# dwofk/fast-depth

Hardware: NVIDIA H100
Metric: depth-maps/sec @224x224 b64 (higher is better)
Workload: dtype f16

## Files before the change

fastdepth_b200/csrc/fd_chain_tc.cu:

```cuda
#include <cuda.h>

#include <cstdio>
#include <cstdlib>
#include <cstring>
#include <new>
#include <string>
#include <vector>

#include "fd_tc_common.cuh"

namespace fd {

constexpr int CH_WORKERS = 16;
constexpr int CH_WARP_TMA = 16;
constexpr int CH_THREADS = 17 * 32;
constexpr int CH_MAX_PASS = 4;
constexpr int CH_MAX_LAYERS = 8, CH_MAX_KB = 8;
constexpr int CH_PITCH = 15, CH_ROWS = 9;
constexpr int CH_BLK = 136 * 128;
constexpr int CH_IN_BYTES = CH_ROWS * CH_PITCH * 128;
constexpr int CH_SB = 4, CH_B_STAGE = 128 * 128;
constexpr int CH_SD = 4, CH_DWP = 9 * 128 + 512;
constexpr int CH_AFF_BYTES = 512 * 8;
constexpr int CH_OFF_ACT = 1024;
constexpr int CH_OFF_B = CH_OFF_ACT + CH_MAX_KB * CH_BLK;
constexpr int CH_OFF_DWP = CH_OFF_B + CH_SB * CH_B_STAGE;
constexpr int CH_OFF_AFF = CH_OFF_DWP + CH_SD * CH_DWP;
constexpr int CH_OFF_BAR = CH_OFF_AFF + 2 * CH_AFF_BYTES;

struct ChainBarriers {
    uint64_t in_full[CH_MAX_KB];
    uint64_t a_full[CH_MAX_KB];
    uint64_t b_full[CH_SB];
    uint64_t b_empty[CH_SB];
    uint64_t dwp_full[CH_SD], dwp_empty[CH_SD];
    uint64_t aff_full[2], aff_empty[2];
    uint64_t mma_done;
    uint64_t halo_full;
    uint64_t act_free;
};
constexpr int CH_SMEM_BYTES = CH_OFF_BAR + (int)sizeof(ChainBarriers) + 1024;

struct ChainLayer {
    int c_in, c_out;
    int kblocks;
    int np;
    int n_pad;
    int aff_bytes;
    const void* dwp;
    const float2* affine;
};

struct ChainParams {
    int n_img, h, w, rows0;
    int n_layers;
    int out_pitch;
    int sleep_ns;
    int n_zero[2];
    void* out;
    ChainLayer L[CH_MAX_LAYERS];
    unsigned long long* trace;
    unsigned char zero_slots[2][48];
};

struct ChainMaps {
    CUtensorMap in;
    CUtensorMap w[CH_MAX_LAYERS];
    CUtensorMap out[2];
};

__device__ __forceinline__ void st_cluster_u32(uint32_t cluster_addr, uint32_t v) {
    asm volatile("st.shared::cluster.b32 [%0], %1;" ::"r"(cluster_addr), "r"(v) : "memory");
}

#define CH_TRACE(row, idx)                                                                                \
    do {                                                                                                  \
        if (p.trace != nullptr && blockIdx.x == 0 && (idx) < 256) p.trace[(row) * 256 + (idx)] = clock64(); \
    } while (0)

template <typename T, bool RELU6>
__global__ void __cluster_dims__(2, 1, 1) __launch_bounds__(CH_THREADS, 1)
chain_tc_kernel(const __grid_constant__ ChainMaps maps, const __grid_constant__ ChainParams p) {
    using MF = MixFma<T>;
    extern __shared__ uint8_t smem_raw[];
    const uint32_t smem_base = (smem_u32(smem_raw) + 1023u) & ~1023u;
    uint8_t* smem = smem_raw + (smem_base - smem_u32(smem_raw));
    ChainBarriers* bars = reinterpret_cast<ChainBarriers*>(smem + CH_OFF_BAR);
    const int warp = threadIdx.x >> 5, lane = threadIdx.x & 31;
    const uint32_t rank = cluster_ctarank();
    const int cluster_id = blockIdx.x >> 1, n_clusters = gridDim.x >> 1;
    const int rows_local = rank == 0 ? p.rows0 : p.h - p.rows0;
    const int row_first = rank == 0 ? 0 : p.rows0;

    if (threadIdx.x == 0) {
        for (int i = 0; i < CH_MAX_KB; ++i) { mbar_init(smem_u32(&bars->in_full[i]), 1); mbar_init(smem_u32(&bars->a_full[i]), CH_WORKERS / 2); }
        for (int i = 0; i < CH_SB; ++i) { mbar_init(smem_u32(&bars->b_full[i]), 1); mbar_init(smem_u32(&bars->b_empty[i]), CH_WORKERS / 4); }
        for (int i = 0; i < CH_SD; ++i) { mbar_init(smem_u32(&bars->dwp_full[i]), 1); mbar_init(smem_u32(&bars->dwp_empty[i]), CH_WORKERS / 2); }
        for (int i = 0; i < 2; ++i) { mbar_init(smem_u32(&bars->aff_full[i]), 1); mbar_init(smem_u32(&bars->aff_empty[i]), CH_WORKERS); }
        mbar_init(smem_u32(&bars->mma_done), 1);
        mbar_init(smem_u32(&bars->halo_full), 1);
        mbar_init(smem_u32(&bars->act_free), 1);
        fence_barrier_init();
    }
    for (int i = threadIdx.x; i < (CH_OFF_B) / 16; i += CH_THREADS) reinterpret_cast<uint4*>(smem)[i] = make_uint4(0u, 0u, 0u, 0u);
    fence_proxy_async();
    if (warp == CH_WARP_TMA && lane == 0) {
        tma_prefetch_desc(&maps.in);
        tma_prefetch_desc(&maps.out[rank]);
        for (int l = 0; l < p.n_layers; ++l) tma_prefetch_desc(&maps.w[l]);
    }
    pdl_launch_dependents();
    pdl_wait_prior_grid();
    cluster_sync_all();

    if (warp == CH_WARP_TMA) {
        if (lane == 0) {
            uint32_t seq = 0;
            for (int img = cluster_id; img < p.n_img; img += n_clusters)
                for (int l = 0; l < p.n_layers; ++l) {
                    const ChainLayer& L = p.L[l];
                    for (int ps = 0; ps < L.np; ++ps)
                        for (int kb = 0; kb < L.kblocks; ++kb, ++seq) {
                            const uint32_t s = seq & (CH_SB - 1), ph = (seq / CH_SB) & 1u;
                            mbar_wait_sleep(smem_u32(&bars->b_empty[s]), ph ^ 1u, (uint32_t)p.sleep_ns);
                            if (kb == 0 && ps == 0 && img == cluster_id) CH_TRACE(10, l);
                            mbar_expect_tx(smem_u32(&bars->b_full[s]), (uint32_t)CH_B_STAGE);
                            tma_load_2d(smem_base + CH_OFF_B + s * CH_B_STAGE, &maps.w[l], smem_u32(&bars->b_full[s]), kb * 64, ps * 128);
                        }
                }
        } else if (lane == 1) {
            uint32_t dseq = 0, lseq = 0;
            for (int img = cluster_id; img < p.n_img; img += n_clusters)
                for (int l = 0; l < p.n_layers; ++l, ++lseq) {
                    const ChainLayer& L = p.L[l];
                    {
                        const uint32_t s = lseq & 1u, ph = (lseq >> 1) & 1u;
                        mbar_wait_sleep(smem_u32(&bars->aff_empty[s]), ph ^ 1u, (uint32_t)p.sleep_ns);
                        mbar_expect_tx(smem_u32(&bars->aff_full[s]), (uint32_t)L.aff_bytes);
                        bulk_load(smem_base + CH_OFF_AFF + s * CH_AFF_BYTES, L.affine, (uint32_t)L.aff_bytes, smem_u32(&bars->aff_full[s]));
                    }
                    for (int kb = 0; kb < L.kblocks; ++kb, ++dseq) {
                        const uint32_t s = dseq & (CH_SD - 1), ph = (dseq / CH_SD) & 1u;
                        mbar_wait_sleep(smem_u32(&bars->dwp_empty[s]), ph ^ 1u, (uint32_t)p.sleep_ns);
                        mbar_expect_tx(smem_u32(&bars->dwp_full[s]), (uint32_t)CH_DWP);
                        bulk_load(smem_base + CH_OFF_DWP + s * CH_DWP, reinterpret_cast<const uint8_t*>(L.dwp) + (size_t)kb * CH_DWP,
                                  (uint32_t)CH_DWP, smem_u32(&bars->dwp_full[s]));
                    }
                }
        } else if (lane == 2) {
            uint32_t it = 0;
            for (int img = cluster_id; img < p.n_img; img += n_clusters, ++it) {
                if (it > 0) mbar_wait_sleep(smem_u32(&bars->act_free), (it - 1u) & 1u, (uint32_t)p.sleep_ns);
                for (int kb = 0; kb < p.L[0].kblocks; ++kb) {
                    mbar_expect_tx(smem_u32(&bars->in_full[kb]), (uint32_t)CH_IN_BYTES);
                    tma_load_4d(smem_base + CH_OFF_ACT + kb * CH_BLK, &maps.in, smem_u32(&bars->in_full[kb]), kb * 64, 0, row_first - 1, img);
                }
            }
        }
    } else {
        const int grp = warp >> 3, wi = warp & 7;
        const bool dw_active = wi < 7;
        const int tx0 = 2 * (dw_active ? wi : 0);
        const int s0 = tx0 - 1;
        uint32_t rd_off[8];
#pragma unroll
        for (int j = 0; j < 8; ++j) rd_off[j] = ((((uint32_t)lane >> 2) ^ ((uint32_t)(s0 + j) & 7u)) << 4) + (((uint32_t)lane & 3u) << 2);
        uint32_t wr_off[2];
#pragma unroll
        for (int ox = 0; ox < 2; ++ox) wr_off[ox] = ((((uint32_t)lane >> 2) ^ ((uint32_t)(tx0 + ox) & 7u)) << 4) + (((uint32_t)lane & 3u) << 2);
        const int nzc = p.n_zero[rank] * 8;
        const uint32_t z_off = (int)threadIdx.x < nzc ? (uint32_t)p.zero_slots[rank][threadIdx.x >> 3] * 128u + ((uint32_t)threadIdx.x & 7u) * 16u : 0u;
        const int rh = (warp >> 2) & 1, ch = warp >> 3, cp = (lane & 3) * 2;
        const bool wg_leader = (warp & 3) == 0 && lane == 0;
        int e_slot[2], e_halo_slot[2], e_last_slot[2];
        bool e_valid[2], e_halo[2];
#pragma unroll
        for (int h = 0; h < 2; ++h) {
            const int m = rh * 64 + (warp & 3) * 16 + (lane >> 2) + 8 * h, e_ty = m >> 4, e_tx = m & 15;
            e_valid[h] = e_ty < rows_local && e_tx < p.w;
            e_slot[h] = (e_ty + 1) * CH_PITCH + e_tx;
            e_last_slot[h] = e_ty * CH_PITCH + e_tx;
            e_halo[h] = e_valid[h] && (rank == 0 ? e_ty == rows_local - 1 : e_ty == 0);
            e_halo_slot[h] = (rank == 0 ? 0 : (p.rows0 + 1) * CH_PITCH) + e_tx;
        }
        const uint32_t peer_act = mapa_u32(smem_base + CH_OFF_ACT, rank ^ 1u);
        const uint32_t peer_halo_full = mapa_u32(smem_u32(&bars->halo_full), rank ^ 1u);
        const uint32_t peer_mma_done = mapa_u32(smem_u32(&bars->mma_done), rank ^ 1u);
        uint32_t dseq_base = 0, lseq = 0, halo_seq = 0, it = 0, bseq = 0, a_par = 0;
        for (int img = cluster_id; img < p.n_img; img += n_clusters, ++it) {
            for (int l = 0; l < p.n_layers; ++l, ++lseq) {
                const ChainLayer& L = p.L[l];
                const bool last = l == p.n_layers - 1;
                const bool tr0 = it == 0 && warp == 0 && lane == 0, tr8 = it == 0 && warp == 8 && lane == 0;
                if (tr0) CH_TRACE(0, l);
                for (int kb = grp; kb < L.kblocks; kb += 2) {
                    uint8_t* blk = smem + CH_OFF_ACT + kb * CH_BLK;
                    if (l == 0) mbar_wait_sleep(smem_u32(&bars->in_full[kb]), it & 1u, (uint32_t)p.sleep_ns);
                    const uint32_t dseq = dseq_base + (uint32_t)kb, ds = dseq & (CH_SD - 1), dph = (dseq / CH_SD) & 1u;
                    mbar_wait(smem_u32(&bars->dwp_full[ds]), dph);
                    const uint8_t* prm = smem + CH_OFF_DWP + ds * CH_DWP;
                    const f32x2 sc = *reinterpret_cast<const f32x2*>(prm + 9 * 128 + lane * 8);
                    const f32x2 bi = *reinterpret_cast<const f32x2*>(prm + 9 * 128 + 256 + lane * 8);
                    const uint8_t* in0 = blk + s0 * 128;
                    uint32_t o[7][2];
                    if (dw_active) {
                        f32x2 acc[7][2];
#pragma unroll
                        for (int a = 0; a < 7; ++a) acc[a][0] = acc[a][1] = 0ull;
                        f32x2 wq[3][3];
#pragma unroll
                        for (int iy = 0; iy < 9; ++iy) {
                            if (iy < 3) {
#pragma unroll
                                for (int kx = 0; kx < 3; ++kx) wq[iy][kx] = MF::widen(*reinterpret_cast<const uint32_t*>(prm + (iy * 3 + kx) * 128 + lane * 4));
                            }
                            f32x2 row[4];
#pragma unroll
                            for (int ix = 0; ix < 4; ++ix) {
                                const int k = iy * CH_PITCH + ix;
                                row[ix] = MF::widen(*reinterpret_cast<const uint32_t*>(in0 + k * 128 + rd_off[k & 7]));
                            }
#pragma unroll
                            for (int oy = 0; oy < 7; ++oy) {
                                const int ky = iy - oy;
                                if (ky < 0 || ky >= 3) continue;
#pragma unroll
                                for (int ox = 0; ox < 2; ++ox)
#pragma unroll
                                    for (int kx = 0; kx < 3; ++kx) ffma2(acc[oy][ox], row[ox + kx], wq[ky][kx]);
                            }
                        }
#pragma unroll
                        for (int oy = 0; oy < 7; ++oy)
#pragma unroll
                            for (int ox = 0; ox < 2; ++ox) o[oy][ox] = MF::template pack_act<RELU6>(ffma2_abc(acc[oy][ox], sc, bi));
                    }
                    __syncwarp();
                    if (tr0 && kb == 0) CH_TRACE(1, l);
                    if (lane == 0) mbar_arrive(smem_u32(&bars->dwp_empty[ds]));
                    asm volatile("bar.sync %0, %1;" ::"r"(1 + grp), "r"(256) : "memory");
                    if (dw_active) {
#pragma unroll
                        for (int oy = 0; oy < 7; ++oy)
#pragma unroll
                            for (int ox = 0; ox < 2; ++ox)
                                *reinterpret_cast<uint32_t*>(blk + (oy * 16 + tx0 + ox) * 128 + wr_off[ox]) = o[oy][ox];
                    }
                    fence_proxy_async();
                    __syncwarp();
                    if (lane == 0) mbar_arrive(smem_u32(&bars->a_full[kb]));
                }
                dseq_base += (uint32_t)L.kblocks;
                if (tr0) CH_TRACE(2, l);
                if (tr8) CH_TRACE(9, l);

                const uint32_t as = lseq & 1u;
                mbar_wait(smem_u32(&bars->aff_full[as]), (lseq >> 1) & 1u);
                const float2* aff = reinterpret_cast<const float2*>(smem + CH_OFF_AFF + as * CH_AFF_BYTES);
                uint32_t pk[CH_MAX_PASS][16];
#pragma unroll
                for (int ps = 0; ps < CH_MAX_PASS; ++ps) {
                    if (ps >= L.np) break;
                    const int col0 = ps * 128 + ch * 64;
                    const bool act = col0 < L.n_pad;
                    float acc[32];
#pragma unroll
                    for (int i = 0; i < 32; ++i) acc[i] = 0.f;
                    for (int kb = 0; kb < L.kblocks; ++kb, ++bseq) {
                        const uint32_t s = bseq & (CH_SB - 1), ph = (bseq / CH_SB) & 1u;
                        mbar_wait(smem_u32(&bars->a_full[kb]), (a_par >> kb) & 1u);
                        mbar_wait(smem_u32(&bars->b_full[s]), ph);
                        if (tr0 && kb == 0 && ps == 0) CH_TRACE(7, l);
                        if (act) {
                            const uint32_t a_lo = sw128_desc_lo(smem_base + CH_OFF_ACT + (uint32_t)kb * CH_BLK + (uint32_t)rh * 8192u);
                            const uint32_t b_lo = sw128_desc_lo(smem_base + CH_OFF_B + s * CH_B_STAGE + (uint32_t)ch * 8192u);
                            wgmma_fence();
#pragma unroll
                            for (int k4 = 0; k4 < 4; ++k4)
                                wgmma_n64<T>(acc, sw128_desc(a_lo + 2u * k4), sw128_desc(b_lo + 2u * k4), (kb > 0 || k4 > 0) ? 1u : 0u);
                            wgmma_commit();
                            wgmma_wait0();
                        }
                        if (wg_leader) mbar_arrive(smem_u32(&bars->b_empty[s]));
                    }
#pragma unroll
                    for (int i = 0; i < 8; ++i) {
                        const int c = col0 + i * 8 + cp;
                        const bool ok = act && col0 + i * 8 < L.n_pad;
                        const float4 af = ok ? *reinterpret_cast<const float4*>(aff + c) : make_float4(0.f, 0.f, 0.f, 0.f);
#pragma unroll
                        for (int h = 0; h < 2; ++h)
                            pk[ps][8 * h + i] = MF::template pack_act<RELU6>(ffma2_abc(f32x2_make(acc[4 * i + 2 * h], acc[4 * i + 2 * h + 1]),
                                                                                        f32x2_make(af.x, af.y), f32x2_make(af.z, af.w)));
                    }
                }
                for (int kb = 0; kb < L.kblocks; ++kb) a_par ^= 1u << kb;
                if (tr0) CH_TRACE(8, l);
                asm volatile("bar.sync %0, %1;" ::"r"(3), "r"(CH_WORKERS * 32) : "memory");
                if (!last) {
                    if (threadIdx.x == 0) mbar_arrive_cluster(peer_mma_done);
                    mbar_wait_cluster(smem_u32(&bars->mma_done), halo_seq & 1u, 0u);
                }
                if (tr0) CH_TRACE(3, l);
#pragma unroll
                for (int ps = 0; ps < CH_MAX_PASS; ++ps) {
                    if (ps >= L.np) break;
                    const int col0 = ps * 128 + ch * 64;
                    if (col0 >= L.n_pad) continue;
                    const uint32_t boff = (uint32_t)(col0 >> 6) * CH_BLK;
#pragma unroll
                    for (int h = 0; h < 2; ++h) {
                        const int w_slot = last ? e_last_slot[h] : e_slot[h];
#pragma unroll
                        for (int i = 0; i < 8; ++i) {
                            if (col0 + i * 8 >= L.n_pad) break;
                            if (e_valid[h])
                                *reinterpret_cast<uint32_t*>(smem + CH_OFF_ACT + boff + w_slot * 128 + (((uint32_t)i ^ ((uint32_t)w_slot & 7u)) << 4) + cp * 2) =
                                    pk[ps][8 * h + i];
                            if (e_halo[h] && !last)
                                st_cluster_u32(peer_act + boff + (uint32_t)e_halo_slot[h] * 128u + (((uint32_t)i ^ ((uint32_t)e_halo_slot[h] & 7u)) << 4) + cp * 2,
                                               pk[ps][8 * h + i]);
                        }
                    }
                }
                if (tr0) CH_TRACE(4, l);
                if (!last) {
                    if ((int)threadIdx.x < nzc) {
                        const int kbn = p.L[l + 1].kblocks;
                        for (int kb = 0; kb < kbn; ++kb)
                            *reinterpret_cast<uint4*>(smem + CH_OFF_ACT + kb * CH_BLK + z_off) = make_uint4(0u, 0u, 0u, 0u);
                    }
                }
                fence_proxy_async();
                __syncwarp();
                if (lane == 0) mbar_arrive(smem_u32(&bars->aff_empty[as]));
                asm volatile("bar.sync %0, %1;" ::"r"(3), "r"(CH_WORKERS * 32) : "memory");
                if (!last && threadIdx.x == 0) mbar_arrive_cluster(peer_halo_full);
                if (tr0) CH_TRACE(5, l);
                if (!last) { mbar_wait_cluster(smem_u32(&bars->halo_full), halo_seq & 1u, 0u); ++halo_seq; }
                if (last && threadIdx.x == 0) {
                    for (int kb = 0; kb < (L.c_out + 63) / 64; ++kb)
                        tma_store_4d(&maps.out[rank], smem_base + CH_OFF_ACT + kb * CH_BLK, kb * 64, 0, row_first, img);
                    bulk_commit_group();
                    bulk_wait_read0();
                    mbar_arrive(smem_u32(&bars->act_free));
                }
                if (tr0) CH_TRACE(6, l);
            }
        }
        if (threadIdx.x == 0) bulk_wait_all();
    }

    __syncwarp();
    cluster_sync_all();
}

template <typename T>
__global__ void chain_pack_dwp_kernel(const float* __restrict__ w, const float* __restrict__ scale, const float* __restrict__ bias,
                                      uint8_t* __restrict__ dst, int c_in, int kblocks) {
    const int i = blockIdx.x * blockDim.x + threadIdx.x;
    if (i >= kblocks * 64) return;
    const int kb = i / 64, cl = i % 64, c = kb * 64 + cl;
    uint8_t* blk = dst + (size_t)kb * CH_DWP;
    T* wt = reinterpret_cast<T*>(blk);
    for (int t = 0; t < 9; ++t) wt[t * 64 + cl] = Traits<T>::from_f(c < c_in ? w[t * c_in + c] : 0.f);
    reinterpret_cast<float*>(blk + 9 * 128)[cl] = c < c_in ? scale[c] : 0.f;
    reinterpret_cast<float*>(blk + 9 * 128 + 256)[cl] = c < c_in ? bias[c] : 0.f;
}
__global__ void chain_pack_affine_kernel(const float* __restrict__ scale, const float* __restrict__ bias, float2* __restrict__ dst,
                                         int n_src, int n_dst) {
    const int i = blockIdx.x * blockDim.x + threadIdx.x;
    if (i < n_dst) {
        const int pair = i >> 1, odd = i & 1;
        float* d = reinterpret_cast<float*>(dst) + pair * 4;
        d[odd] = i < n_src ? scale[i] : 0.f;
        d[2 + odd] = i < n_src ? bias[i] : 0.f;
    }
}

struct ChainTcPlan {
    ChainMaps maps;
    ChainParams p;
    dim3 grid;
    int dtype, relu6;
    TcLaunchOpts opts;
    std::vector<void*> owned;
    size_t owned_bytes = 0;
    std::string name;
};

bool chain_tc_supported(int dtype, const StageGeom* g, int n_layers) {
    if (dtype != FD_F16 && dtype != FD_BF16) return false;
    if (n_layers < 2 || n_layers > CH_MAX_LAYERS) return false;
    if (get_tensor_map_encoder() == nullptr) return false;
    for (int i = 0; i < n_layers; ++i) {
        const StageGeom& s = g[i];
        if (s.ksize != 3 || s.stride != 1 || s.upsample) return false;
        if (s.c_in % 8 || s.c_out % 8 || s.c_in > 512 || s.c_out > 512) return false;
        if (s.h_out != g[0].h_out || s.w_out != g[0].w_out || s.h_in != s.h_out || s.w_in != s.w_out) return false;
        if (s.act != g[0].act) return false;
        if (i > 0 && s.c_in != g[i - 1].c_out) return false;
        if (i > 0 && s.in_pitch > 0 && s.in_pitch != s.c_in) return false;
    }
    const int h = g[0].h_out, w = g[0].w_out;
    return h >= 2 && h <= 14 && w >= 1 && w <= 14;
}

void chain_tc_destroy(ChainTcPlan* cp) {
    if (!cp) return;
    for (void* q : cp->owned) cudaFree(q);
    delete cp;
}
const char* chain_tc_name(ChainTcPlan* cp) { return cp->name.c_str(); }
size_t chain_tc_param_bytes(ChainTcPlan* cp) { return cp->owned_bytes; }

int chain_tc_prepare(int dtype, const BlockArgs* layers, int n_layers, const TcLaunchOpts& opts, ChainTcPlan** out) {
    PFN_encodeTiled encode = get_tensor_map_encoder();
    if (!encode) return fail(FD_ERR_CUDA, "cuTensorMapEncodeTiled is not available from this driver");
    ChainTcPlan* cp = new (std::nothrow) ChainTcPlan();
    if (!cp) return fail(FD_ERR_CUDA, "out of host memory");
    cp->dtype = dtype; cp->opts = opts; cp->relu6 = layers[0].g.act == FD_ACT_RELU6;
    ChainParams& p = cp->p;
    memset(&p, 0, sizeof(p));
    memset(&cp->maps, 0, sizeof(cp->maps));
    const StageGeom& g0 = layers[0].g;
    p.n_img = g0.n; p.h = g0.h_out; p.w = g0.w_out; p.rows0 = (p.h + 1) / 2; p.n_layers = n_layers;
    p.sleep_ns = opts.sleep_ns;
    const StageGeom& gl = layers[n_layers - 1].g;
    p.out = layers[n_layers - 1].out;
    p.out_pitch = gl.out_pitch > 0 ? gl.out_pitch : gl.c_out;
    for (int r = 0; r < 2; ++r) {
        const int rows_local = r == 0 ? p.rows0 : p.h - p.rows0;
        int nz = 0;
        auto add = [&](int slot) {
            for (int i = 0; i < nz; ++i) if (p.zero_slots[r][i] == slot) return;
            p.zero_slots[r][nz++] = (unsigned char)slot;
        };
        for (int rr = 0; rr <= rows_local + 1; ++rr) { add(rr * CH_PITCH + p.w); add(rr * CH_PITCH + CH_PITCH - 1); }
        const int border = r == 0 ? 0 : rows_local + 1;
        for (int c = 0; c < p.w; ++c) add(border * CH_PITCH + c);
        p.n_zero[r] = nz;
    }
    const size_t es = 2;
    const CUtensorMapDataType dt = dtype == FD_F16 ? CU_TENSOR_MAP_DATA_TYPE_FLOAT16 : CU_TENSOR_MAP_DATA_TYPE_BFLOAT16;
    int rc = FD_OK;
    for (int l = 0; l < n_layers && rc == FD_OK; ++l) {
        const StageGeom& g = layers[l].g;
        ChainLayer& L = p.L[l];
        L.c_in = g.c_in; L.c_out = g.c_out;
        L.kblocks = (g.c_in + 63) / 64;
        L.n_pad = (g.c_out + 63) / 64 * 64;
        L.np = (L.n_pad + 127) / 128;
        L.aff_bytes = L.n_pad * 8;
        void* dwp = nullptr; float2* aff = nullptr;
        if (cudaMalloc(&dwp, (size_t)L.kblocks * CH_DWP) != cudaSuccess || cudaMalloc(&aff, (size_t)L.n_pad * sizeof(float2)) != cudaSuccess) {
            cudaFree(dwp); rc = fail(FD_ERR_CUDA, "cudaMalloc failed"); break;
        }
        cp->owned.push_back(dwp); cp->owned.push_back(aff);
        cp->owned_bytes += (size_t)L.kblocks * CH_DWP + (size_t)L.n_pad * sizeof(float2);
        const int tot = L.kblocks * 64;
        if (dtype == FD_F16) chain_pack_dwp_kernel<__half><<<(tot + 127) / 128, 128>>>(layers[l].dw_w, layers[l].dw_scale, layers[l].dw_bias, (uint8_t*)dwp, g.c_in, L.kblocks);
        else chain_pack_dwp_kernel<__nv_bfloat16><<<(tot + 127) / 128, 128>>>(layers[l].dw_w, layers[l].dw_scale, layers[l].dw_bias, (uint8_t*)dwp, g.c_in, L.kblocks);
        chain_pack_affine_kernel<<<(L.n_pad + 127) / 128, 128>>>(layers[l].pw_scale, layers[l].pw_bias, aff, g.c_out, L.n_pad);
        if (cudaGetLastError() != cudaSuccess) { rc = fail(FD_ERR_CUDA, "chain parameter packing launch failed"); break; }
        L.dwp = dwp; L.affine = aff;
        cuuint64_t dims[2] = {(cuuint64_t)g.c_in, (cuuint64_t)g.c_out};
        cuuint64_t strides[1] = {(cuuint64_t)g.c_in * es};
        cuuint32_t box[2] = {64, 128};
        cuuint32_t estr[2] = {1, 1};
        CUresult r = encode(&cp->maps.w[l], dt, 2, const_cast<void*>(layers[l].pw_w), dims, strides, box, estr, CU_TENSOR_MAP_INTERLEAVE_NONE,
                            CU_TENSOR_MAP_SWIZZLE_128B, CU_TENSOR_MAP_L2_PROMOTION_L2_256B, CU_TENSOR_MAP_FLOAT_OOB_FILL_NONE);
        if (r != CUDA_SUCCESS) rc = fail(FD_ERR_CUDA, "cuTensorMapEncodeTiled(chain weights) failed: " + std::to_string((int)r));
    }
    if (rc == FD_OK && cudaDeviceSynchronize() != cudaSuccess) rc = fail(FD_ERR_CUDA, "chain parameter packing failed");
    if (rc == FD_OK) {
        const int in_pitch = g0.in_pitch > 0 ? g0.in_pitch : g0.c_in;
        cuuint64_t dims[4] = {(cuuint64_t)g0.c_in, (cuuint64_t)g0.w_in, (cuuint64_t)g0.h_in, (cuuint64_t)g0.n};
        cuuint64_t strides[3] = {(cuuint64_t)in_pitch * es, (cuuint64_t)g0.w_in * in_pitch * es, (cuuint64_t)g0.h_in * g0.w_in * in_pitch * es};
        cuuint32_t box[4] = {64, (cuuint32_t)CH_PITCH, (cuuint32_t)CH_ROWS, 1};
        cuuint32_t estr[4] = {1, 1, 1, 1};
        CUresult r = encode(&cp->maps.in, dt, 4, const_cast<void*>(layers[0].in), dims, strides, box, estr, CU_TENSOR_MAP_INTERLEAVE_NONE,
                            CU_TENSOR_MAP_SWIZZLE_128B, CU_TENSOR_MAP_L2_PROMOTION_L2_128B, CU_TENSOR_MAP_FLOAT_OOB_FILL_NONE);
        if (r != CUDA_SUCCESS) rc = fail(FD_ERR_CUDA, "cuTensorMapEncodeTiled(chain input) failed: " + std::to_string((int)r));
    }
    for (int r = 0; r < 2 && rc == FD_OK; ++r) {
        const int rows_r = r == 0 ? p.rows0 : p.h - p.rows0;
        const cuuint64_t P = (cuuint64_t)p.out_pitch;
        cuuint64_t dims[4] = {(cuuint64_t)gl.c_out, (cuuint64_t)gl.w_out, (cuuint64_t)gl.h_out, (cuuint64_t)gl.n};
        cuuint64_t strides[3] = {P * es, (cuuint64_t)gl.w_out * P * es, (cuuint64_t)gl.h_out * gl.w_out * P * es};
        cuuint32_t box[4] = {64, (cuuint32_t)CH_PITCH, (cuuint32_t)rows_r, 1};
        cuuint32_t estr[4] = {1, 1, 1, 1};
        CUresult cr = encode(&cp->maps.out[r], dt, 4, p.out, dims, strides, box, estr, CU_TENSOR_MAP_INTERLEAVE_NONE,
                             CU_TENSOR_MAP_SWIZZLE_128B, CU_TENSOR_MAP_L2_PROMOTION_L2_128B, CU_TENSOR_MAP_FLOAT_OOB_FILL_NONE);
        if (cr != CUDA_SUCCESS) rc = fail(FD_ERR_CUDA, "cuTensorMapEncodeTiled(chain output) failed: " + std::to_string((int)cr));
    }
    if (rc != FD_OK) { chain_tc_destroy(cp); return rc; }
    const int clusters = std::min(p.n_img, std::max(1, opts.n_sms / 2));
    cp->grid = dim3((unsigned)(2 * clusters), 1, 1);
    char buf[160];
    snprintf(buf, sizeof(buf), "chain_tc<k3,s1,2cta>[%d layers,%dx%d,c%d..%d,kb%d,smem%dK]", n_layers, p.h, p.w, p.L[0].c_in, p.L[n_layers - 1].c_out,
             p.L[0].kblocks, CH_SMEM_BYTES / 1024);
    cp->name = buf;
    *out = cp;
    return FD_OK;
}

template <typename T, bool RELU6>
static int chain_launch_inst(ChainTcPlan* cp, cudaStream_t st) {
    auto kern = chain_tc_kernel<T, RELU6>;
    static PerDeviceOnce attr_set;
    int dev = -1;
    FD_CUDA_OK(cudaGetDevice(&dev));
    if (attr_set.need(dev)) {
        FD_CUDA_OK(cudaFuncSetAttribute(kern, cudaFuncAttributeMaxDynamicSharedMemorySize, CH_SMEM_BYTES));
        attr_set.done(dev);
    }
    cudaLaunchConfig_t cfg{};
    cfg.gridDim = cp->grid; cfg.blockDim = dim3(CH_THREADS); cfg.dynamicSmemBytes = CH_SMEM_BYTES; cfg.stream = st;
    cudaLaunchAttribute attr[1];
    attr[0].id = cudaLaunchAttributeProgrammaticStreamSerialization;
    attr[0].val.programmaticStreamSerializationAllowed = 1;
    cfg.attrs = attr; cfg.numAttrs = cp->opts.pdl ? 1 : 0;
    FD_CUDA_OK(cudaLaunchKernelEx(&cfg, kern, cp->maps, cp->p));
    FD_CUDA_OK(cudaGetLastError());
    return FD_OK;
}

int chain_tc_launch(ChainTcPlan* cp, cudaStream_t st);
int chain_tc_trace(ChainTcPlan* cp, cudaStream_t st, unsigned long long* out_host, int* rows, int* cols) {
    unsigned long long* dev = nullptr;
    const size_t bytes = 12 * 256 * sizeof(unsigned long long);
    FD_CUDA_OK(cudaMalloc(&dev, bytes));
    FD_CUDA_OK(cudaMemsetAsync(dev, 0, bytes, st));
    cp->p.trace = dev;
    int rc = chain_tc_launch(cp, st);
    cp->p.trace = nullptr;
    if (rc == FD_OK && cudaStreamSynchronize(st) != cudaSuccess) rc = fail(FD_ERR_CUDA, "chain trace run failed");
    if (rc == FD_OK) cudaMemcpy(out_host, dev, bytes, cudaMemcpyDeviceToHost);
    cudaFree(dev);
    *rows = 12; *cols = 256;
    return rc;
}

int chain_tc_launch(ChainTcPlan* cp, cudaStream_t st) {
    if (cp->dtype == FD_F16) return cp->relu6 ? chain_launch_inst<__half, true>(cp, st) : chain_launch_inst<__half, false>(cp, st);
    return cp->relu6 ? chain_launch_inst<__nv_bfloat16, true>(cp, st) : chain_launch_inst<__nv_bfloat16, false>(cp, st);
}

}
```

fastdepth_b200/plan.py:

```python
import ctypes

import numpy as np
import torch
import torch.nn as nn

from . import _lib
from ._lib import StageDesc

DTYPE_CODE = {torch.float32: _lib.FD_F32, torch.float16: _lib.FD_F16, torch.bfloat16: _lib.FD_BF16}
N_METRICS = 11
METRIC_NAMES = ('irmse', 'imae', 'mse', 'rmse', 'mae', 'absrel', 'lg10', 'delta1', 'delta2', 'delta3')

SKIP_FOR_DECODE = {2: 5, 3: 3, 4: 1}


def fold_bn(bn):
    g = bn.weight.detach().float().cpu()
    b = bn.bias.detach().float().cpu()
    m = bn.running_mean.detach().float().cpu()
    v = bn.running_var.detach().float().cpu()
    scale = g / torch.sqrt(v + float(bn.eps))
    bias = b - m * scale
    return scale.contiguous().numpy(), bias.contiguous().numpy()


def _act_of(m):
    if isinstance(m, nn.ReLU6):
        return _lib.FD_ACT_RELU6
    if isinstance(m, nn.ReLU):
        return _lib.FD_ACT_RELU
    raise RuntimeError('unsupported activation %r on the hot path' % type(m).__name__)


def _w(conv):
    return np.ascontiguousarray(conv.weight.detach().float().cpu().numpy())


def _sq(v):
    return int(v[0]) if isinstance(v, (tuple, list)) else int(v)


def _blocks_of(module):
    if hasattr(module, 'conv0') and hasattr(module, 'decode_conv6'):
        enc = [getattr(module, 'conv%d' % i) for i in range(14)]
        dec = [getattr(module, 'decode_conv%d' % j) for j in range(1, 6)]
        names = ['conv%d' % i for i in range(14)] + ['decode_conv%d' % j for j in range(1, 7)]
        concat = type(module).__name__ == 'MobileNetSkipConcat' or \
            dec[2][0][0].weight.shape[0] != dec[1][1][0].weight.shape[0]
        return enc, dec, module.decode_conv6, ('concat' if concat else True), names
    if hasattr(module, 'mobilenet') and hasattr(module, 'decoder'):
        enc = [module.mobilenet[i] for i in range(14)]
        for child in ('convt', 'upconv'):
            if hasattr(module.decoder, child + '1'):
                dec = [getattr(module.decoder, '%s%d' % (child, j)) for j in range(1, 6)]
                names = ['mobilenet.%d' % i for i in range(14)] + ['decoder.%s%d' % (child, j) for j in range(1, 6)]
                return enc, dec, module.decoder.convf, False, names + ['decoder.convf']
        dec = [getattr(module.decoder, 'conv%d' % j) for j in range(1, 6)]
        names = ['mobilenet.%d' % i for i in range(14)] + ['decoder.conv%d' % j for j in range(1, 7)]
        return enc, dec, module.decoder.conv6, False, names
    raise RuntimeError('unsupported module for the fastdepth_b200 hot path: %s' % type(module).__name__)


def _is_dense_block(b):
    return (isinstance(b, nn.Sequential) and len(b) == 3 and isinstance(b[0], nn.Conv2d) and b[0].groups == 1 and
            _sq(b[0].kernel_size) in (3, 5) and _sq(b[0].stride) == 1 and isinstance(b[1], nn.BatchNorm2d))


def _convt_kind(b):
    if not isinstance(b, nn.Sequential):
        return None
    if len(b) == 3 and isinstance(b[0], nn.ConvTranspose2d) and isinstance(b[1], nn.BatchNorm2d):
        c, k = b[0], _sq(b[0].kernel_size)
        ok = (k in (3, 5, 7, 9) and c.groups == 1 and _sq(c.stride) == 2 and _sq(c.padding) == (k - 1) // 2 and
              _sq(c.output_padding) == 1 and _sq(c.dilation) == 1 and c.bias is None)
        return _lib.FD_STAGE_DECONV if ok else None
    if len(b) == 4 and type(b[0]).__name__ == 'Unpool' and isinstance(b[1], nn.Conv2d) and isinstance(b[2], nn.BatchNorm2d):
        c = b[1]
        ok = (getattr(b[0], 'stride', None) == 2 and _sq(c.kernel_size) == 5 and c.groups == 1 and _sq(c.stride) == 1 and
              _sq(c.padding) == 2 and _sq(c.dilation) == 1 and c.bias is None)
        return _lib.FD_STAGE_UPCONV if ok else None
    return None


def dense_decoder(module):
    try:
        _, dec, _, _, _ = _blocks_of(module)
        return all(_is_dense_block(b) for b in dec) or all(_convt_kind(b) is not None for b in dec)
    except Exception:
        return False


def supports(module):
    try:
        enc, dec, head, _, _ = _blocks_of(module)
        return all(isinstance(b, nn.Sequential) and len(b) == 2 and isinstance(b[0], nn.Sequential) and
                   b[0][0].groups == b[0][0].in_channels for b in dec) or dense_decoder(module)
    except Exception:
        return False


def describe(module):
    enc, dec, hd, with_skips, names = _blocks_of(module)
    descs, weights = [], []
    conv0 = enc[0]
    c, bn, act = conv0[0], conv0[1], conv0[2]
    descs.append(dict(kind=_lib.FD_STAGE_STEM, c_in=c.weight.shape[1], c_out=c.weight.shape[0],
                      ksize=_sq(c.kernel_size), stride=_sq(c.stride), act=_act_of(act), upsample=0, skip_src=-1))
    s, b = fold_bn(bn)
    weights.append((None, None, None, _w(c), s, b))
    stage_of_encoder = {0: 0}
    for i in range(1, 14):
        blk = enc[i]
        dw, bn1, a1, pw, bn2, a2 = blk[0], blk[1], blk[2], blk[3], blk[4], blk[5]
        if _act_of(a1) != _act_of(a2):
            raise RuntimeError('encoder block %d: mixed activations are not supported' % i)
        descs.append(dict(kind=_lib.FD_STAGE_DWPW, c_in=dw.weight.shape[0], c_out=pw.weight.shape[0],
                          ksize=_sq(dw.kernel_size), stride=_sq(dw.stride), act=_act_of(a1), upsample=0, skip_src=-1))
        s1, b1 = fold_bn(bn1)
        s2, b2 = fold_bn(bn2)
        weights.append((_w(dw).reshape(dw.weight.shape[0], -1), s1, b1,
                        _w(pw).reshape(pw.weight.shape[0], pw.weight.shape[1]), s2, b2))
        stage_of_encoder[i] = len(descs) - 1
    for j in range(1, 6):
        blk = dec[j - 1]
        kind = _convt_kind(blk)
        if kind is not None:
            c, bn, a = (blk[0], blk[1], blk[2]) if kind == _lib.FD_STAGE_DECONV else (blk[1], blk[2], blk[3])
            c_in, c_out = (c.weight.shape[0], c.weight.shape[1]) if kind == _lib.FD_STAGE_DECONV else \
                (c.weight.shape[1], c.weight.shape[0])
            descs.append(dict(kind=kind, c_in=c_in, c_out=c_out, ksize=_sq(c.kernel_size), stride=2, act=_act_of(a),
                              upsample=0, skip_src=-1))
            s, b = fold_bn(bn)
            weights.append((None, None, None, _w(c).reshape(c.weight.shape[0], -1), s, b))
            continue
        if _is_dense_block(blk):
            c, bn, a = blk[0], blk[1], blk[2]
            descs.append(dict(kind=_lib.FD_STAGE_CONV, c_in=c.weight.shape[1], c_out=c.weight.shape[0],
                              ksize=_sq(c.kernel_size), stride=1, act=_act_of(a), upsample=1, skip_src=-1))
            s, b = fold_bn(bn)
            weights.append((None, None, None, _w(c).reshape(c.weight.shape[0], -1), s, b))
            continue
        (dw, bn1, a1), (pw, bn2, a2) = (blk[0][0], blk[0][1], blk[0][2]), (blk[1][0], blk[1][1], blk[1][2])
        if _act_of(a1) != _act_of(a2):
            raise RuntimeError('decoder block %d: mixed activations are not supported' % j)
        skip = stage_of_encoder[SKIP_FOR_DECODE[j]] if (with_skips and j in SKIP_FOR_DECODE) else -1
        descs.append(dict(kind=_lib.FD_STAGE_DWPW, c_in=dw.weight.shape[0], c_out=pw.weight.shape[0],
                          ksize=_sq(dw.kernel_size), stride=1, act=_act_of(a1), upsample=1, skip_src=skip,
                          skip_mode=1 if (with_skips == 'concat' and skip >= 0) else 0))
        s1, b1 = fold_bn(bn1)
        s2, b2 = fold_bn(bn2)
        weights.append((_w(dw).reshape(dw.weight.shape[0], -1), s1, b1,
                        _w(pw).reshape(pw.weight.shape[0], pw.weight.shape[1]), s2, b2))
    c, bn, act = hd[0], hd[1], hd[2]
    descs.append(dict(kind=_lib.FD_STAGE_HEAD, c_in=c.weight.shape[1], c_out=1, ksize=1, stride=1,
                      act=_act_of(act), upsample=0, skip_src=-1))
    s, b = fold_bn(bn)
    weights.append((None, None, None, _w(c).reshape(1, -1), s, b))
    return descs, weights, names


def _fp(a):
    if a is None:
        return None
    assert a.dtype == np.float32 and a.flags['C_CONTIGUOUS']
    return a.ctypes.data_as(ctypes.c_void_p)


class Plan:

    def __init__(self, descs, weights, names, n, h, w, dtype, device_index):
        self.lib = _lib.load()
        self.n, self.h, self.w, self.dtype = n, h, w, dtype
        self.device_index = device_index
        self.names = list(names)
        arr = (StageDesc * len(descs))(*[StageDesc(**d) for d in descs])
        handle = ctypes.c_void_p()
        _lib.check(self.lib.fd_plan_create(arr, len(descs), n, h, w, DTYPE_CODE[dtype], device_index,
                                           ctypes.byref(handle)))
        self.handle = handle
        self.set_weights(weights)

    @classmethod
    def from_module(cls, module, n, h, w, dtype, device_index):
        descs, weights, names = describe(module)
        return cls(descs, weights, names, n, h, w, dtype, device_index)

    def set_weights(self, weights):
        for i, wt in enumerate(weights):
            keep = [np.ascontiguousarray(a, dtype=np.float32) if a is not None else None for a in wt]
            _lib.check(self.lib.fd_plan_set_stage_weights(self.handle, i, *[_fp(a) for a in keep]))

    def set_option(self, name, value):
        _lib.check(self.lib.fd_plan_set_option(self.handle, name.encode(), int(value)))

    def get_option(self, name):
        v = ctypes.c_int()
        _lib.check(self.lib.fd_plan_get_option(self.handle, name.encode(), ctypes.byref(v)))
        return v.value

    def forward(self, x, y, stream_ptr, n=None):
        n = x.shape[0] if n is None else int(n)
        _lib.check(self.lib.fd_forward_shape(self.handle, n, x.shape[2], x.shape[3], x.data_ptr(), y.data_ptr(),
                                             stream_ptr))

    def forward_host(self, x_host, y_host, stream_ptr):
        _lib.check(self.lib.fd_forward_host(self.handle, x_host.data_ptr(), y_host.data_ptr(), stream_ptr))

    def pipeline_submit(self, x_host, y_host):
        t = ctypes.c_uint64()
        _lib.check(self.lib.fd_pipeline_submit(self.handle, x_host.data_ptr(), y_host.data_ptr(), ctypes.byref(t)))
        return t.value

    def pipeline_wait(self, ticket):
        _lib.check(self.lib.fd_pipeline_wait(self.handle, ticket))

    def launches_per_forward(self):
        v = ctypes.c_int()
        _lib.check(self.lib.fd_plan_launches_per_forward(self.handle, ctypes.byref(v)))
        return v.value

    def workspace_bytes(self):
        v = ctypes.c_size_t()
        _lib.check(self.lib.fd_plan_workspace_bytes(self.handle, ctypes.byref(v)))
        return v.value

    def steps(self):
        n = ctypes.c_int()
        _lib.check(self.lib.fd_plan_step_count(self.handle, ctypes.byref(n)))
        out = []
        for i in range(n.value):
            st, ab, mc = ctypes.c_int(), ctypes.c_double(), ctypes.c_double()
            buf = ctypes.create_string_buffer(200)
            _lib.check(self.lib.fd_plan_step_info(self.handle, i, ctypes.byref(st), ctypes.byref(ab), ctypes.byref(mc),
                                                  buf, 200))
            dwm, dnm = ctypes.c_double(), ctypes.c_double()
            _lib.check(self.lib.fd_plan_step_macs(self.handle, i, ctypes.byref(dwm), ctypes.byref(dnm)))
            kname = buf.value.decode()
            sname = self.names[st.value]
            if 'chain_tc' in kname and '{stages ' in kname:
                a, b = kname.split('{stages ')[1].rstrip('}').split('-')
                sname = '%s..%s' % (self.names[int(a)], self.names[int(b)])
            out.append(dict(step=i, stage=st.value, stage_name=sname, kernel=kname,
                            alg_bytes=ab.value, macs=mc.value, dw_macs=dwm.value, dense_macs=dnm.value))
        return out

    def time_steps(self, x, y, stream_ptr, warmup=3, iters=20, flush_l2=True):
        steps = self.steps()
        ms = (ctypes.c_float * len(steps))()
        _lib.check(self.lib.fd_plan_time_steps(self.handle, x.data_ptr(), y.data_ptr(), stream_ptr, warmup, iters,
                                               1 if flush_l2 else 0, ms))
        for s, t in zip(steps, ms):
            s['ms'] = float(t)
        return steps

    def trace_stage(self, stage, y, stream_ptr):
        import numpy as np
        buf = (ctypes.c_uint64 * 3072)()
        rows, cols = ctypes.c_int(), ctypes.c_int()
        _lib.check(self.lib.fd_plan_trace_stage(self.handle, stage, y.data_ptr(), stream_ptr, buf, 3072,
                                                ctypes.byref(rows), ctypes.byref(cols)))
        a = np.frombuffer(buf, dtype=np.uint64).reshape(rows.value, cols.value).astype(np.int64)
        in_chain = False
        for st in self.steps():
            if 'chain_tc' in st['kernel'] and '{stages ' in st['kernel']:
                lo, hi = st['kernel'].split('{stages ')[1].rstrip('}').split('-')
                in_chain = in_chain or int(lo) <= stage <= int(hi)
        if in_chain:
            cnames = ('layer_start', 'dw_first_kb_computed', 'dw_done_grp0', 'pointwise_done', 'epilogue_done', 'local_barrier',
                      'halo_received', 'mma_first_a_full', 'mma_last_pass_done', 'dw_done_grp1', 'tma_first_b_issue', 'unused11')
            return {n: a[i][a[i] > 0] for i, n in enumerate(cnames)}
        names = ('tma_issue', 'dw_start', 'dw_math_done', 'a_published', 'mma_ready', 'mma_issued', 'unused6', 'epi_done',
                 'unused8', 'epi_staged', 'epi_barrier', 'epi_store_issued')
        return {n: a[i][a[i] > 0] for i, n in enumerate(names)}

    def stage_tensor(self, stage, which=0):
        ptr = ctypes.c_void_p()
        n, h, w, c, cs = (ctypes.c_int() for _ in range(5))
        _lib.check(self.lib.fd_stage_buffer(self.handle, stage, which, ctypes.byref(ptr), ctypes.byref(n),
                                            ctypes.byref(h), ctypes.byref(w), ctypes.byref(c), ctypes.byref(cs)))
        numel = (n.value * h.value * w.value - 1) * cs.value + c.value
        flat = _alias_device_memory(ptr.value, (numel,), numel, self.dtype, self.device_index)
        return flat.as_strided((n.value, h.value, w.value, c.value),
                               (h.value * w.value * cs.value, w.value * cs.value, cs.value, 1))

    def close(self):
        if getattr(self, 'handle', None):
            self.lib.fd_plan_destroy(self.handle)
            self.handle = None

    def __del__(self):
        try:
            self.close()
        except Exception:
            pass


class _CudaArrayView:

    def __init__(self, ptr, shape, typestr):
        self.__cuda_array_interface__ = {'data': (ptr, False), 'shape': shape, 'typestr': typestr, 'version': 3,
                                         'strides': None}


def _alias_device_memory(ptr, shape, numel, dtype, device_index):
    if dtype == torch.float32:
        with torch.cuda.device(device_index):
            return torch.as_tensor(_CudaArrayView(ptr, (numel,), '<f4'), device='cuda:%d' % device_index).view(shape)
    with torch.cuda.device(device_index):
        raw = torch.as_tensor(_CudaArrayView(ptr, (numel,), '<i2'), device='cuda:%d' % device_index)
    return raw.view(dtype).view(shape)


def metrics_accumulate(pred, target, sums):
    lib = _lib.load()
    assert pred.is_cuda and target.is_cuda and sums.is_cuda and sums.dtype == torch.float64 and sums.numel() == N_METRICS
    pred = pred.contiguous()
    target = target.contiguous().float()
    n = pred.shape[0]
    hw = pred[0].numel()
    stream = torch.cuda.current_stream(pred.device).cuda_stream
    _lib.check(lib.fd_metrics_accumulate(pred.data_ptr(), target.data_ptr(), DTYPE_CODE[pred.dtype], n, hw,
                                         sums.data_ptr(), pred.device.index, stream))
```

Baseline: 58290.

## Split chain kernel across variable-size cluster with 4-row tiles and multicast weights

Restructures the fused depthwise+pointwise chain kernel. It moves from a fixed 2-CTA cluster splitting rows in half to a cluster of ceil(h/4) CTAs, each owning 4 output rows. It uses dedicated depthwise warps, warpgroup-wide MMA over 256-row weight tiles multicast across the cluster, and halo exchange with up and down neighbours. Grid size now comes from the occupancy API. This is meant to spread each image across more SMs and cut per-CTA weight traffic, at the cost of more cross-CTA synchronisation and halo traffic.

```diff
diff --git a/fastdepth_b200/csrc/fd_chain_tc.cu b/fastdepth_b200/csrc/fd_chain_tc.cu
--- a/fastdepth_b200/csrc/fd_chain_tc.cu
+++ b/fastdepth_b200/csrc/fd_chain_tc.cu
@@ -1,5 +1,6 @@
 #include <cuda.h>
 
+#include <algorithm>
 #include <cstdio>
 #include <cstdlib>
 #include <cstring>
@@ -11,15 +12,14 @@
 
 namespace fd {
 
-constexpr int CH_WORKERS = 16;
-constexpr int CH_WARP_TMA = 16;
-constexpr int CH_THREADS = 17 * 32;
-constexpr int CH_MAX_PASS = 4;
-constexpr int CH_MAX_LAYERS = 8, CH_MAX_KB = 8;
-constexpr int CH_PITCH = 15, CH_ROWS = 9;
-constexpr int CH_BLK = 136 * 128;
+constexpr int CH_THREADS = 3 * 128;
+constexpr int CH_DW_WARPS = 2, CH_WG_MMA = 1;
+constexpr int CH_MAX_LAYERS = 8, CH_MAX_KB = 8, CH_MAX_CLUSTER = 4;
+constexpr int CH_TILE_ROWS = 4;
+constexpr int CH_PITCH = 15, CH_ROWS = CH_TILE_ROWS + 2;
+constexpr int CH_BLK = 96 * 128;
 constexpr int CH_IN_BYTES = CH_ROWS * CH_PITCH * 128;
-constexpr int CH_SB = 4, CH_B_STAGE = 128 * 128;
+constexpr int CH_SB = 3, CH_B_ROWS = 256, CH_B_STAGE = CH_B_ROWS * 128;
 constexpr int CH_SD = 4, CH_DWP = 9 * 128 + 512;
 constexpr int CH_AFF_BYTES = 512 * 8;
 constexpr int CH_OFF_ACT = 1024;
@@ -27,6 +27,9 @@
 constexpr int CH_OFF_DWP = CH_OFF_B + CH_SB * CH_B_STAGE;
 constexpr int CH_OFF_AFF = CH_OFF_DWP + CH_SD * CH_DWP;
 constexpr int CH_OFF_BAR = CH_OFF_AFF + 2 * CH_AFF_BYTES;
+static_assert(CH_BLK % 1024 == 0 && CH_OFF_ACT % 1024 == 0 && CH_OFF_B % 1024 == 0 && CH_B_STAGE % 1024 == 0, "SW128 tiles need 1 KB alignment");
+static_assert(CH_ROWS * CH_PITCH < CH_BLK / 128, "each block needs a spare zero slot after its pixels");
+static_assert(64 * 128 <= CH_BLK, "the m64 operand tile is written in place over its block");
 
 struct ChainBarriers {
     uint64_t in_full[CH_MAX_KB];
@@ -35,40 +38,48 @@
     uint64_t b_empty[CH_SB];
     uint64_t dwp_full[CH_SD], dwp_empty[CH_SD];
     uint64_t aff_full[2], aff_empty[2];
+    uint64_t act_full;
     uint64_t mma_done;
     uint64_t halo_full;
     uint64_t act_free;
 };
 constexpr int CH_SMEM_BYTES = CH_OFF_BAR + (int)sizeof(ChainBarriers) + 1024;
+static_assert(CH_SMEM_BYTES <= 227 * 1024, "chain kernel shared memory exceeds the 227 KB opt-in limit");
 
 struct ChainLayer {
     int c_in, c_out;
     int kblocks;
-    int np;
     int n_pad;
+    int ncw;
     int aff_bytes;
     const void* dwp;
     const float2* affine;
 };
 
 struct ChainParams {
-    int n_img, h, w, rows0;
+    int n_img, h, w;
+    int cl;
     int n_layers;
-    int out_pitch;
     int sleep_ns;
-    int n_zero[2];
-    void* out;
+    int n_zero[CH_MAX_CLUSTER];
     ChainLayer L[CH_MAX_LAYERS];
     unsigned long long* trace;
-    unsigned char zero_slots[2][48];
+    unsigned char zero_slots[CH_MAX_CLUSTER][48];
 };
 
 struct ChainMaps {
     CUtensorMap in;
     CUtensorMap w[CH_MAX_LAYERS];
-    CUtensorMap out[2];
+    CUtensorMap out[CH_MAX_CLUSTER];
 };
 
+__device__ __forceinline__ void acc_fence(float (&d)[128]) {
+#pragma unroll
+    for (int i = 0; i < 128; ++i) asm volatile("" : "+f"(d[i])::"memory");
+}
+__device__ __forceinline__ void mbar_arrive_remote(uint32_t cluster_addr) {
+    asm volatile("mbarrier.arrive.shared::cluster.b64 _, [%0];" ::"r"(cluster_addr) : "memory");
+}
 __device__ __forceinline__ void st_cluster_u32(uint32_t cluster_addr, uint32_t v) {
     asm volatile("st.shared::cluster.b32 [%0], %1;" ::"r"(cluster_addr), "r"(v) : "memory");
 }
@@ -79,32 +90,36 @@
     } while (0)
 
 template <typename T, bool RELU6>
-__global__ void __cluster_dims__(2, 1, 1) __launch_bounds__(CH_THREADS, 1)
+__global__ void __launch_bounds__(CH_THREADS, 1)
 chain_tc_kernel(const __grid_constant__ ChainMaps maps, const __grid_constant__ ChainParams p) {
     using MF = MixFma<T>;
     extern __shared__ uint8_t smem_raw[];
     const uint32_t smem_base = (smem_u32(smem_raw) + 1023u) & ~1023u;
     uint8_t* smem = smem_raw + (smem_base - smem_u32(smem_raw));
     ChainBarriers* bars = reinterpret_cast<ChainBarriers*>(smem + CH_OFF_BAR);
-    const int warp = threadIdx.x >> 5, lane = threadIdx.x & 31;
+    const int warp = threadIdx.x >> 5, lane = threadIdx.x & 31, wg = warp >> 2;
+    const uint32_t cl = (uint32_t)p.cl;
     const uint32_t rank = cluster_ctarank();
-    const int cluster_id = blockIdx.x >> 1, n_clusters = gridDim.x >> 1;
-    const int rows_local = rank == 0 ? p.rows0 : p.h - p.rows0;
-    const int row_first = rank == 0 ? 0 : p.rows0;
+    const int cluster_id = blockIdx.x / p.cl, n_clusters = gridDim.x / p.cl;
+    const int row_first = 4 * (int)rank;
+    const int rows_local = min(CH_TILE_ROWS, p.h - row_first);
+    const bool has_up = rank > 0, has_dn = rank + 1 < cl;
+    const uint32_t n_nbr = (has_up ? 1u : 0u) + (has_dn ? 1u : 0u);
 
     if (threadIdx.x == 0) {
-        for (int i = 0; i < CH_MAX_KB; ++i) { mbar_init(smem_u32(&bars->in_full[i]), 1); mbar_init(smem_u32(&bars->a_full[i]), CH_WORKERS / 2); }
-        for (int i = 0; i < CH_SB; ++i) { mbar_init(smem_u32(&bars->b_full[i]), 1); mbar_init(smem_u32(&bars->b_empty[i]), CH_WORKERS / 4); }
-        for (int i = 0; i < CH_SD; ++i) { mbar_init(smem_u32(&bars->dwp_full[i]), 1); mbar_init(smem_u32(&bars->dwp_empty[i]), CH_WORKERS / 2); }
-        for (int i = 0; i < 2; ++i) { mbar_init(smem_u32(&bars->aff_full[i]), 1); mbar_init(smem_u32(&bars->aff_empty[i]), CH_WORKERS); }
-        mbar_init(smem_u32(&bars->mma_done), 1);
-        mbar_init(smem_u32(&bars->halo_full), 1);
+        for (int i = 0; i < CH_MAX_KB; ++i) { mbar_init(smem_u32(&bars->in_full[i]), 1); mbar_init(smem_u32(&bars->a_full[i]), CH_DW_WARPS); }
+        for (int i = 0; i < CH_SB; ++i) { mbar_init(smem_u32(&bars->b_full[i]), 1); mbar_init(smem_u32(&bars->b_empty[i]), cl); }
+        for (int i = 0; i < CH_SD; ++i) { mbar_init(smem_u32(&bars->dwp_full[i]), 1); mbar_init(smem_u32(&bars->dwp_empty[i]), CH_DW_WARPS); }
+        for (int i = 0; i < 2; ++i) { mbar_init(smem_u32(&bars->aff_full[i]), 1); mbar_init(smem_u32(&bars->aff_empty[i]), 8); }
+        mbar_init(smem_u32(&bars->act_full), 8);
+        mbar_init(smem_u32(&bars->mma_done), n_nbr > 0 ? n_nbr : 1u);
+        mbar_init(smem_u32(&bars->halo_full), n_nbr > 0 ? n_nbr : 1u);
         mbar_init(smem_u32(&bars->act_free), 1);
         fence_barrier_init();
     }
-    for (int i = threadIdx.x; i < (CH_OFF_B) / 16; i += CH_THREADS) reinterpret_cast<uint4*>(smem)[i] = make_uint4(0u, 0u, 0u, 0u);
+    for (int i = threadIdx.x; i < CH_OFF_B / 16; i += CH_THREADS) reinterpret_cast<uint4*>(smem)[i] = make_uint4(0u, 0u, 0u, 0u);
     fence_proxy_async();
-    if (warp == CH_WARP_TMA && lane == 0) {
+    if (threadIdx.x == 0) {
         tma_prefetch_desc(&maps.in);
         tma_prefetch_desc(&maps.out[rank]);
         for (int l = 0; l < p.n_layers; ++l) tma_prefetch_desc(&maps.w[l]);
@@ -113,22 +128,26 @@
     pdl_wait_prior_grid();
     cluster_sync_all();
 
-    if (warp == CH_WARP_TMA) {
-        if (lane == 0) {
-            uint32_t seq = 0;
+    if (warp >= CH_DW_WARPS && wg == 0) {
+        if (warp == CH_DW_WARPS && lane == 0) {
+            const uint16_t mask = (uint16_t)((1u << cl) - 1u);
+            Ring rb;
+            uint32_t t = 0;
             for (int img = cluster_id; img < p.n_img; img += n_clusters)
                 for (int l = 0; l < p.n_layers; ++l) {
                     const ChainLayer& L = p.L[l];
-                    for (int ps = 0; ps < L.np; ++ps)
-                        for (int kb = 0; kb < L.kblocks; ++kb, ++seq) {
-                            const uint32_t s = seq & (CH_SB - 1), ph = (seq / CH_SB) & 1u;
-                            mbar_wait_sleep(smem_u32(&bars->b_empty[s]), ph ^ 1u, (uint32_t)p.sleep_ns);
-                            if (kb == 0 && ps == 0 && img == cluster_id) CH_TRACE(10, l);
-                            mbar_expect_tx(smem_u32(&bars->b_full[s]), (uint32_t)CH_B_STAGE);
-                            tma_load_2d(smem_base + CH_OFF_B + s * CH_B_STAGE, &maps.w[l], smem_u32(&bars->b_full[s]), kb * 64, ps * 128);
+                    for (int kb = 0; kb < L.kblocks; ++kb)
+                        for (int cw = 0; cw < L.ncw; ++cw, ++t) {
+                            mbar_wait_sleep(smem_u32(&bars->b_empty[rb.s]), rb.ph ^ 1u, (uint32_t)p.sleep_ns);
+                            if (kb == 0 && cw == 0 && img == cluster_id) CH_TRACE(10, l);
+                            const uint32_t bar = smem_u32(&bars->b_full[rb.s]), dst = smem_base + CH_OFF_B + rb.s * CH_B_STAGE;
+                            mbar_expect_tx(bar, (uint32_t)CH_B_STAGE);
+                            if (cl == 1) tma_load_2d(dst, &maps.w[l], bar, kb * 64, cw * CH_B_ROWS);
+                            else if (t % cl == rank) tma_load_2d_multicast(dst, &maps.w[l], bar, kb * 64, cw * CH_B_ROWS, mask);
+                            rb.next(CH_SB);
                         }
                 }
-        } else if (lane == 1) {
+        } else if (warp == CH_DW_WARPS + 1 && lane == 0) {
             uint32_t dseq = 0, lseq = 0;
             for (int img = cluster_id; img < p.n_img; img += n_clusters)
                 for (int l = 0; l < p.n_layers; ++l, ++lseq) {
@@ -147,7 +166,7 @@
                                   (uint32_t)CH_DWP, smem_u32(&bars->dwp_full[s]));
                     }
                 }
-        } else if (lane == 2) {
+        } else if (warp == CH_DW_WARPS && lane == 1) {
             uint32_t it = 0;
             for (int img = cluster_id; img < p.n_img; img += n_clusters, ++it) {
                 if (it > 0) mbar_wait_sleep(smem_u32(&bars->act_free), (it - 1u) & 1u, (uint32_t)p.sleep_ns);
@@ -157,176 +176,169 @@
                 }
             }
         }
+    } else if (warp < CH_DW_WARPS) {
+        const int oy0 = 2 * warp;
+        const bool act0 = oy0 < rows_local, act1 = oy0 + 1 < rows_local;
+        const int s0 = oy0 * CH_PITCH - 1;
+        uint32_t rd_off[8];
+#pragma unroll
+        for (int j = 0; j < 8; ++j) rd_off[j] = ((((uint32_t)lane >> 2) ^ ((uint32_t)(s0 + j) & 7u)) << 4) + (((uint32_t)lane & 3u) << 2);
+        const uint32_t lane_w = ((uint32_t)lane & 3u) << 2;
+        uint32_t dseq = 0, hs = 0, it = 0;
+        for (int img = cluster_id; img < p.n_img; img += n_clusters, ++it) {
+            for (int l = 0; l < p.n_layers; ++l) {
+                const ChainLayer& L = p.L[l];
+                const bool trc = it == 0 && warp == 0 && lane == 0;
+                if (trc) CH_TRACE(0, l);
+                if (l > 0) {
+                    mbar_wait(smem_u32(&bars->act_full), hs & 1u);
+                    if (n_nbr) mbar_wait_cluster(smem_u32(&bars->halo_full), hs & 1u, 0u);
+                    ++hs;
+                }
+                if (trc) CH_TRACE(1, l);
+                for (int kb = 0; kb < L.kblocks; ++kb, ++dseq) {
+                    uint8_t* blk = smem + CH_OFF_ACT + kb * CH_BLK;
+                    if (l == 0) mbar_wait(smem_u32(&bars->in_full[kb]), it & 1u);
+                    const uint32_t ds = dseq & (CH_SD - 1), dph = (dseq / CH_SD) & 1u;
+                    mbar_wait(smem_u32(&bars->dwp_full[ds]), dph);
+                    const uint8_t* prm = smem + CH_OFF_DWP + ds * CH_DWP;
+                    uint32_t o[2][14];
+                    if (act0) {
+                        f32x2 wq[3][3];
+#pragma unroll
+                        for (int t9 = 0; t9 < 9; ++t9) wq[t9 / 3][t9 % 3] = MF::widen(*reinterpret_cast<const uint32_t*>(prm + t9 * 128 + lane * 4));
+                        f32x2 acc[2][14];
+#pragma unroll
+                        for (int ox = 0; ox < 14; ++ox) acc[0][ox] = acc[1][ox] = 0ull;
+                        const uint8_t* in0 = blk + s0 * 128;
+#pragma unroll
+                        for (int iy = 0; iy < 4; ++iy)
+#pragma unroll
+                            for (int ix = 0; ix < 16; ++ix) {
+                                const int k = iy * CH_PITCH + ix;
+                                const f32x2 v = MF::widen(*reinterpret_cast<const uint32_t*>(in0 + k * 128 + rd_off[k & 7]));
+#pragma unroll
+                                for (int oy = 0; oy < 2; ++oy) {
+                                    const int ky = iy - oy;
+                                    if (ky < 0 || ky > 2) continue;
+#pragma unroll
+                                    for (int kx = 0; kx < 3; ++kx) {
+                                        const int ox = ix - kx;
+                                        if (ox >= 0 && ox < 14) ffma2(acc[oy][ox], v, wq[ky][kx]);
+                                    }
+                                }
+                            }
+                        const f32x2 sc = *reinterpret_cast<const f32x2*>(prm + 9 * 128 + lane * 8);
+                        const f32x2 bi = *reinterpret_cast<const f32x2*>(prm + 9 * 128 + 256 + lane * 8);
+#pragma unroll
+                        for (int oy = 0; oy < 2; ++oy)
+#pragma unroll
+                            for (int ox = 0; ox < 14; ++ox) o[oy][ox] = MF::template pack_act<RELU6>(ffma2_abc(acc[oy][ox], sc, bi));
+                    }
+                    __syncwarp();
+                    if (lane == 0) mbar_arrive(smem_u32(&bars->dwp_empty[ds]));
+                    asm volatile("bar.sync 1, %0;" ::"n"(CH_DW_WARPS * 32) : "memory");
+#pragma unroll
+                    for (int oy = 0; oy < 2; ++oy) {
+                        if (oy == 0 ? !act0 : !act1) continue;
+#pragma unroll
+                        for (int ox = 0; ox < 14; ++ox)
+                            *reinterpret_cast<uint32_t*>(blk + (16 * (oy0 + oy) + ox) * 128 + ((((uint32_t)lane >> 2) ^ ((uint32_t)ox & 7u)) << 4) + lane_w) =
+                                o[oy][ox];
+                    }
+                    fence_proxy_async();
+                    __syncwarp();
+                    if (lane == 0) mbar_arrive(smem_u32(&bars->a_full[kb]));
+                    if (trc && kb == 0) CH_TRACE(2, l);
+                }
+                if (trc) CH_TRACE(3, l);
+            }
+        }
     } else {
-        const int grp = warp >> 3, wi = warp & 7;
-        const bool dw_active = wi < 7;
-        const int tx0 = 2 * (dw_active ? wi : 0);
-        const int s0 = tx0 - 1;
-        uint32_t rd_off[8];
-#pragma unroll
-        for (int j = 0; j < 8; ++j) rd_off[j] = ((((uint32_t)lane >> 2) ^ ((uint32_t)(s0 + j) & 7u)) << 4) + (((uint32_t)lane & 3u) << 2);
-        uint32_t wr_off[2];
-#pragma unroll
-        for (int ox = 0; ox < 2; ++ox) wr_off[ox] = ((((uint32_t)lane >> 2) ^ ((uint32_t)(tx0 + ox) & 7u)) << 4) + (((uint32_t)lane & 3u) << 2);
+        const int cw = wg - CH_WG_MMA;
+        const int ct = (int)threadIdx.x - 128 * CH_WG_MMA;
+        const int wq = warp & 3;
+        const int cp = (lane & 3) * 2;
+        const bool row_valid = wq < rows_local;
+        const bool halo_up = has_up && wq == 0, halo_dn = has_dn && wq == rows_local - 1;
+        const uint32_t up_act = mapa_u32(smem_base + CH_OFF_ACT, rank - (has_up ? 1u : 0u));
+        const uint32_t dn_act = mapa_u32(smem_base + CH_OFF_ACT, rank + (has_dn ? 1u : 0u));
         const int nzc = p.n_zero[rank] * 8;
-        const uint32_t z_off = (int)threadIdx.x < nzc ? (uint32_t)p.zero_slots[rank][threadIdx.x >> 3] * 128u + ((uint32_t)threadIdx.x & 7u) * 16u : 0u;
-        const int rh = (warp >> 2) & 1, ch = warp >> 3, cp = (lane & 3) * 2;
-        const bool wg_leader = (warp & 3) == 0 && lane == 0;
-        int e_slot[2], e_halo_slot[2], e_last_slot[2];
-        bool e_valid[2], e_halo[2];
-#pragma unroll
-        for (int h = 0; h < 2; ++h) {
-            const int m = rh * 64 + (warp & 3) * 16 + (lane >> 2) + 8 * h, e_ty = m >> 4, e_tx = m & 15;
-            e_valid[h] = e_ty < rows_local && e_tx < p.w;
-            e_slot[h] = (e_ty + 1) * CH_PITCH + e_tx;
-            e_last_slot[h] = e_ty * CH_PITCH + e_tx;
-            e_halo[h] = e_valid[h] && (rank == 0 ? e_ty == rows_local - 1 : e_ty == 0);
-            e_halo_slot[h] = (rank == 0 ? 0 : (p.rows0 + 1) * CH_PITCH) + e_tx;
-        }
-        const uint32_t peer_act = mapa_u32(smem_base + CH_OFF_ACT, rank ^ 1u);
-        const uint32_t peer_halo_full = mapa_u32(smem_u32(&bars->halo_full), rank ^ 1u);
-        const uint32_t peer_mma_done = mapa_u32(smem_u32(&bars->mma_done), rank ^ 1u);
-        uint32_t dseq_base = 0, lseq = 0, halo_seq = 0, it = 0, bseq = 0, a_par = 0;
+        Ring rb;
+        uint32_t lseq = 0, hs = 0, it = 0, a_par = 0;
         for (int img = cluster_id; img < p.n_img; img += n_clusters, ++it) {
             for (int l = 0; l < p.n_layers; ++l, ++lseq) {
                 const ChainLayer& L = p.L[l];
                 const bool last = l == p.n_layers - 1;
-                const bool tr0 = it == 0 && warp == 0 && lane == 0, tr8 = it == 0 && warp == 8 && lane == 0;
-                if (tr0) CH_TRACE(0, l);
-                for (int kb = grp; kb < L.kblocks; kb += 2) {
-                    uint8_t* blk = smem + CH_OFF_ACT + kb * CH_BLK;
-                    if (l == 0) mbar_wait_sleep(smem_u32(&bars->in_full[kb]), it & 1u, (uint32_t)p.sleep_ns);
-                    const uint32_t dseq = dseq_base + (uint32_t)kb, ds = dseq & (CH_SD - 1), dph = (dseq / CH_SD) & 1u;
-                    mbar_wait(smem_u32(&bars->dwp_full[ds]), dph);
-                    const uint8_t* prm = smem + CH_OFF_DWP + ds * CH_DWP;
-                    const f32x2 sc = *reinterpret_cast<const f32x2*>(prm + 9 * 128 + lane * 8);
-                    const f32x2 bi = *reinterpret_cast<const f32x2*>(prm + 9 * 128 + 256 + lane * 8);
-                    const uint8_t* in0 = blk + s0 * 128;
-                    uint32_t o[7][2];
-                    if (dw_active) {
-                        f32x2 acc[7][2];
-#pragma unroll
-                        for (int a = 0; a < 7; ++a) acc[a][0] = acc[a][1] = 0ull;
-                        f32x2 wq[3][3];
-#pragma unroll
-                        for (int iy = 0; iy < 9; ++iy) {
-                            if (iy < 3) {
-#pragma unroll
-                                for (int kx = 0; kx < 3; ++kx) wq[iy][kx] = MF::widen(*reinterpret_cast<const uint32_t*>(prm + (iy * 3 + kx) * 128 + lane * 4));
-                            }
-                            f32x2 row[4];
-#pragma unroll
-                            for (int ix = 0; ix < 4; ++ix) {
-                                const int k = iy * CH_PITCH + ix;
-                                row[ix] = MF::widen(*reinterpret_cast<const uint32_t*>(in0 + k * 128 + rd_off[k & 7]));
-                            }
-#pragma unroll
-                            for (int oy = 0; oy < 7; ++oy) {
-                                const int ky = iy - oy;
-                                if (ky < 0 || ky >= 3) continue;
-#pragma unroll
-                                for (int ox = 0; ox < 2; ++ox)
-#pragma unroll
-                                    for (int kx = 0; kx < 3; ++kx) ffma2(acc[oy][ox], row[ox + kx], wq[ky][kx]);
-                            }
-                        }
-#pragma unroll
-                        for (int oy = 0; oy < 7; ++oy)
-#pragma unroll
-                            for (int ox = 0; ox < 2; ++ox) o[oy][ox] = MF::template pack_act<RELU6>(ffma2_abc(acc[oy][ox], sc, bi));
-                    }
-                    __syncwarp();
-                    if (tr0 && kb == 0) CH_TRACE(1, l);
-                    if (lane == 0) mbar_arrive(smem_u32(&bars->dwp_empty[ds]));
-                    asm volatile("bar.sync %0, %1;" ::"r"(1 + grp), "r"(256) : "memory");
-                    if (dw_active) {
-#pragma unroll
-                        for (int oy = 0; oy < 7; ++oy)
-#pragma unroll
-                            for (int ox = 0; ox < 2; ++ox)
-                                *reinterpret_cast<uint32_t*>(blk + (oy * 16 + tx0 + ox) * 128 + wr_off[ox]) = o[oy][ox];
-                    }
-                    fence_proxy_async();
-                    __syncwarp();
-                    if (lane == 0) mbar_arrive(smem_u32(&bars->a_full[kb]));
-                }
-                dseq_base += (uint32_t)L.kblocks;
-                if (tr0) CH_TRACE(2, l);
-                if (tr8) CH_TRACE(9, l);
-
+                const bool trc = it == 0 && ct == 0, trc1 = it == 0 && ct == 128;
+                const bool act = cw < L.ncw;
+                float acc[128];
+                if (act) {
+#pragma unroll
+                    for (int i = 0; i < 128; ++i) acc[i] = 0.f;
+                    acc_fence(acc);
+                    uint32_t prev_s = 0;
+                    for (int kb = 0; kb < L.kblocks; ++kb) {
+                        if (cw == 1) rb.next(CH_SB);
+                        const uint32_t s = rb.s;
+                        mbar_wait(smem_u32(&bars->a_full[kb]), (a_par >> kb) & 1u);
+                        mbar_wait(smem_u32(&bars->b_full[s]), rb.ph);
+                        if (trc && kb == 0) CH_TRACE(4, l);
+                        const uint32_t a_lo = sw128_desc_lo(smem_base + CH_OFF_ACT + (uint32_t)kb * CH_BLK);
+                        const uint32_t b_lo = sw128_desc_lo(smem_base + CH_OFF_B + s * CH_B_STAGE);
+                        wgmma_fence();
+#pragma unroll
+                        for (int k4 = 0; k4 < 4; ++k4)
+                            wgmma_n256<T>(acc, sw128_desc(a_lo + 2u * k4), sw128_desc(b_lo + 2u * k4), (kb > 0 || k4 > 0) ? 1u : 0u);
+                        wgmma_commit();
+                        wgmma_wait1();
+                        acc_fence(acc);
+                        if (kb > 0 && wq == 0 && (uint32_t)lane < cl) mbar_arrive_remote(mapa_u32(smem_u32(&bars->b_empty[prev_s]), (uint32_t)lane));
+                        prev_s = s;
+                        rb.next(CH_SB);
+                        if (cw == 0 && L.ncw == 2) rb.next(CH_SB);
+                    }
+                    wgmma_wait0();
+                    acc_fence(acc);
+                    if (wq == 0 && (uint32_t)lane < cl) mbar_arrive_remote(mapa_u32(smem_u32(&bars->b_empty[prev_s]), (uint32_t)lane));
+                } else {
+                    for (int kb = 0; kb < L.kblocks; ++kb) rb.next(CH_SB);
+                }
+                for (int kb = 0; kb < L.kblocks; ++kb) a_par ^= 1u << kb;
+                if (trc) CH_TRACE(5, l);
+                if (trc1) CH_TRACE(9, l);
+                asm volatile("bar.sync 2, 256;" ::: "memory");
+                if (!last && n_nbr && ct == 0) {
+                    if (has_up) mbar_arrive_cluster(mapa_u32(smem_u32(&bars->mma_done), rank - 1u));
+                    if (has_dn) mbar_arrive_cluster(mapa_u32(smem_u32(&bars->mma_done), rank + 1u));
+                }
+                if (trc) CH_TRACE(6, l);
                 const uint32_t as = lseq & 1u;
                 mbar_wait(smem_u32(&bars->aff_full[as]), (lseq >> 1) & 1u);
                 const float2* aff = reinterpret_cast<const float2*>(smem + CH_OFF_AFF + as * CH_AFF_BYTES);
-                uint32_t pk[CH_MAX_PASS][16];
-#pragma unroll
-                for (int ps = 0; ps < CH_MAX_PASS; ++ps) {
-                    if (ps >= L.np) break;
-                    const int col0 = ps * 128 + ch * 64;
-                    const bool act = col0 < L.n_pad;
-                    float acc[32];
-#pragma unroll
-                    for (int i = 0; i < 32; ++i) acc[i] = 0.f;
-                    for (int kb = 0; kb < L.kblocks; ++kb, ++bseq) {
-                        const uint32_t s = bseq & (CH_SB - 1), ph = (bseq / CH_SB) & 1u;
-                        mbar_wait(smem_u32(&bars->a_full[kb]), (a_par >> kb) & 1u);
-                        mbar_wait(smem_u32(&bars->b_full[s]), ph);
-                        if (tr0 && kb == 0 && ps == 0) CH_TRACE(7, l);
-                        if (act) {
-                            const uint32_t a_lo = sw128_desc_lo(smem_base + CH_OFF_ACT + (uint32_t)kb * CH_BLK + (uint32_t)rh * 8192u);
-                            const uint32_t b_lo = sw128_desc_lo(smem_base + CH_OFF_B + s * CH_B_STAGE + (uint32_t)ch * 8192u);
-                            wgmma_fence();
-#pragma unroll
-                            for (int k4 = 0; k4 < 4; ++k4)
-                                wgmma_n64<T>(acc, sw128_desc(a_lo + 2u * k4), sw128_desc(b_lo + 2u * k4), (kb > 0 || k4 > 0) ? 1u : 0u);
-                            wgmma_commit();
-                            wgmma_wait0();
+                if (act) {
+#pragma unroll
+                    for (int j = 0; j < 32; ++j) {
+                        const int c = 256 * cw + 8 * j;
+                        if (c >= L.n_pad) break;
+                        const float4 af = *reinterpret_cast<const float4*>(aff + c + cp);
+                        const uint32_t boff = (uint32_t)(c >> 6) * CH_BLK;
+#pragma unroll
+                        for (int h = 0; h < 2; ++h) {
+                            const uint32_t v = MF::template pack_act<RELU6>(ffma2_abc(f32x2_make(acc[4 * j + 2 * h], acc[4 * j + 2 * h + 1]),
+                                                                                      f32x2_make(af.x, af.y), f32x2_make(af.z, af.w)));
+                            acc[4 * j + 2 * h] = __uint_as_float(v);
+                            const int tx = (lane >> 2) + 8 * h;
+                            const int slot = last ? wq * CH_PITCH + tx : (wq + 1) * CH_PITCH + tx;
+                            if (row_valid && tx < p.w)
+                                *reinterpret_cast<uint32_t*>(smem + CH_OFF_ACT + boff + slot * 128 + ((((uint32_t)j & 7u) ^ ((uint32_t)slot & 7u)) << 4) + cp * 2) = v;
                         }
-                        if (wg_leader) mbar_arrive(smem_u32(&bars->b_empty[s]));
-                    }
-#pragma unroll
-                    for (int i = 0; i < 8; ++i) {
-                        const int c = col0 + i * 8 + cp;
-                        const bool ok = act && col0 + i * 8 < L.n_pad;
-                        const float4 af = ok ? *reinterpret_cast<const float4*>(aff + c) : make_float4(0.f, 0.f, 0.f, 0.f);
-#pragma unroll
-                        for (int h = 0; h < 2; ++h)
-                            pk[ps][8 * h + i] = MF::template pack_act<RELU6>(ffma2_abc(f32x2_make(acc[4 * i + 2 * h], acc[4 * i + 2 * h + 1]),
-                                                                                        f32x2_make(af.x, af.y), f32x2_make(af.z, af.w)));
-                    }
-                }
-                for (int kb = 0; kb < L.kblocks; ++kb) a_par ^= 1u << kb;
-                if (tr0) CH_TRACE(8, l);
-                asm volatile("bar.sync %0, %1;" ::"r"(3), "r"(CH_WORKERS * 32) : "memory");
+                    }
+                }
                 if (!last) {
-                    if (threadIdx.x == 0) mbar_arrive_cluster(peer_mma_done);
-                    mbar_wait_cluster(smem_u32(&bars->mma_done), halo_seq & 1u, 0u);
-                }
-                if (tr0) CH_TRACE(3, l);
-#pragma unroll
-                for (int ps = 0; ps < CH_MAX_PASS; ++ps) {
-                    if (ps >= L.np) break;
-                    const int col0 = ps * 128 + ch * 64;
-                    if (col0 >= L.n_pad) continue;
-                    const uint32_t boff = (uint32_t)(col0 >> 6) * CH_BLK;
-#pragma unroll
-                    for (int h = 0; h < 2; ++h) {
-                        const int w_slot = last ? e_last_slot[h] : e_slot[h];
-#pragma unroll
-                        for (int i = 0; i < 8; ++i) {
-                            if (col0 + i * 8 >= L.n_pad) break;
-                            if (e_valid[h])
-                                *reinterpret_cast<uint32_t*>(smem + CH_OFF_ACT + boff + w_slot * 128 + (((uint32_t)i ^ ((uint32_t)w_slot & 7u)) << 4) + cp * 2) =
-                                    pk[ps][8 * h + i];
-                            if (e_halo[h] && !last)
-                                st_cluster_u32(peer_act + boff + (uint32_t)e_halo_slot[h] * 128u + (((uint32_t)i ^ ((uint32_t)e_halo_slot[h] & 7u)) << 4) + cp * 2,
-                                               pk[ps][8 * h + i]);
-                        }
-                    }
-                }
-                if (tr0) CH_TRACE(4, l);
-                if (!last) {
-                    if ((int)threadIdx.x < nzc) {
-                        const int kbn = p.L[l + 1].kblocks;
+                    const int kbn = p.L[l + 1].kblocks;
+                    for (int z = ct; z < nzc; z += 256) {
+                        const uint32_t z_off = (uint32_t)p.zero_slots[rank][z >> 3] * 128u + ((uint32_t)z & 7u) * 16u;
                         for (int kb = 0; kb < kbn; ++kb)
                             *reinterpret_cast<uint4*>(smem + CH_OFF_ACT + kb * CH_BLK + z_off) = make_uint4(0u, 0u, 0u, 0u);
                     }
@@ -334,21 +346,49 @@
                 fence_proxy_async();
                 __syncwarp();
                 if (lane == 0) mbar_arrive(smem_u32(&bars->aff_empty[as]));
-                asm volatile("bar.sync %0, %1;" ::"r"(3), "r"(CH_WORKERS * 32) : "memory");
-                if (!last && threadIdx.x == 0) mbar_arrive_cluster(peer_halo_full);
-                if (tr0) CH_TRACE(5, l);
-                if (!last) { mbar_wait_cluster(smem_u32(&bars->halo_full), halo_seq & 1u, 0u); ++halo_seq; }
-                if (last && threadIdx.x == 0) {
-                    for (int kb = 0; kb < (L.c_out + 63) / 64; ++kb)
-                        tma_store_4d(&maps.out[rank], smem_base + CH_OFF_ACT + kb * CH_BLK, kb * 64, 0, row_first, img);
-                    bulk_commit_group();
-                    bulk_wait_read0();
-                    mbar_arrive(smem_u32(&bars->act_free));
-                }
-                if (tr0) CH_TRACE(6, l);
+                if (!last && lane == 0) mbar_arrive(smem_u32(&bars->act_full));
+                if (trc) CH_TRACE(7, l);
+                if (!last && n_nbr) {
+                    if (act && (halo_up || halo_dn)) {
+                        mbar_wait_cluster(smem_u32(&bars->mma_done), hs & 1u, 0u);
+#pragma unroll
+                        for (int j = 0; j < 32; ++j) {
+                            const int c = 256 * cw + 8 * j;
+                            if (c >= L.n_pad) break;
+                            const uint32_t boff = (uint32_t)(c >> 6) * CH_BLK;
+#pragma unroll
+                            for (int h = 0; h < 2; ++h) {
+                                const int tx = (lane >> 2) + 8 * h;
+                                if (tx >= p.w) continue;
+                                const uint32_t v = __float_as_uint(acc[4 * j + 2 * h]);
+                                const uint32_t sup = (uint32_t)((CH_ROWS - 1) * CH_PITCH + tx), sdn = (uint32_t)tx;
+                                if (halo_up) st_cluster_u32(up_act + boff + sup * 128u + ((((uint32_t)j & 7u) ^ (sup & 7u)) << 4) + cp * 2, v);
+                                if (halo_dn) st_cluster_u32(dn_act + boff + sdn * 128u + ((((uint32_t)j & 7u) ^ (sdn & 7u)) << 4) + cp * 2, v);
+                            }
+                        }
+                    }
+                    asm volatile("bar.sync 2, 256;" ::: "memory");
+                    if (ct == 0) {
+                        if (has_up) mbar_arrive_cluster(mapa_u32(smem_u32(&bars->halo_full), rank - 1u));
+                        if (has_dn) mbar_arrive_cluster(mapa_u32(smem_u32(&bars->halo_full), rank + 1u));
+                    }
+                }
+                if (!last) ++hs;
+                if (trc) CH_TRACE(8, l);
+                if (last) {
+                    asm volatile("bar.sync 2, 256;" ::: "memory");
+                    if (ct == 0) {
+                        for (int kb = 0; kb < (L.c_out + 63) / 64; ++kb)
+                            tma_store_4d(&maps.out[rank], smem_base + CH_OFF_ACT + kb * CH_BLK, kb * 64, 0, row_first, img);
+                        bulk_commit_group();
+                        bulk_wait_read0();
+                        mbar_arrive(smem_u32(&bars->act_free));
+                    }
+                }
+                if (trc) CH_TRACE(11, l);
             }
         }
-        if (threadIdx.x == 0) bulk_wait_all();
+        if (ct == 0) bulk_wait_all();
     }
 
     __syncwarp();
@@ -414,6 +454,41 @@
 const char* chain_tc_name(ChainTcPlan* cp) { return cp->name.c_str(); }
 size_t chain_tc_param_bytes(ChainTcPlan* cp) { return cp->owned_bytes; }
 
+template <typename T, bool RELU6>
+static int chain_kernel_ready() {
+    static PerDeviceOnce attr_set;
+    int dev = -1;
+    FD_CUDA_OK(cudaGetDevice(&dev));
+    if (attr_set.need(dev)) {
+        FD_CUDA_OK(cudaFuncSetAttribute(chain_tc_kernel<T, RELU6>, cudaFuncAttributeMaxDynamicSharedMemorySize, CH_SMEM_BYTES));
+        attr_set.done(dev);
+    }
+    return FD_OK;
+}
+static void chain_config(ChainTcPlan* cp, cudaStream_t st, cudaLaunchConfig_t& cfg, cudaLaunchAttribute (&attr)[2]) {
+    cfg = cudaLaunchConfig_t{};
+    cfg.gridDim = cp->grid; cfg.blockDim = dim3(CH_THREADS); cfg.dynamicSmemBytes = CH_SMEM_BYTES; cfg.stream = st;
+    attr[0].id = cudaLaunchAttributeClusterDimension;
+    attr[0].val.clusterDim.x = (unsigned)cp->p.cl; attr[0].val.clusterDim.y = 1; attr[0].val.clusterDim.z = 1;
+    attr[1].id = cudaLaunchAttributeProgrammaticStreamSerialization;
+    attr[1].val.programmaticStreamSerializationAllowed = 1;
+    cfg.attrs = attr; cfg.numAttrs = cp->opts.pdl ? 2 : 1;
+}
+template <typename T, bool RELU6>
+static int chain_size_grid(ChainTcPlan* cp) {
+    int rc = chain_kernel_ready<T, RELU6>();
+    if (rc != FD_OK) return rc;
+    cudaLaunchConfig_t cfg;
+    cudaLaunchAttribute attr[2];
+    cp->grid = dim3((unsigned)(cp->p.n_img * cp->p.cl), 1, 1);
+    chain_config(cp, nullptr, cfg, attr);
+    int n_cl = 0;
+    FD_CUDA_OK(cudaOccupancyMaxActiveClusters(&n_cl, chain_tc_kernel<T, RELU6>, &cfg));
+    if (n_cl < 1) return fail(FD_ERR_UNSUPPORTED, "chain kernel: no cluster of " + std::to_string(cp->p.cl) + " CTAs fits the device");
+    cp->grid = dim3((unsigned)(std::min(n_cl, cp->p.n_img) * cp->p.cl), 1, 1);
+    return FD_OK;
+}
+
 int chain_tc_prepare(int dtype, const BlockArgs* layers, int n_layers, const TcLaunchOpts& opts, ChainTcPlan** out) {
     PFN_encodeTiled encode = get_tensor_map_encoder();
     if (!encode) return fail(FD_ERR_CUDA, "cuTensorMapEncodeTiled is not available from this driver");
@@ -424,21 +499,22 @@
     memset(&p, 0, sizeof(p));
     memset(&cp->maps, 0, sizeof(cp->maps));
     const StageGeom& g0 = layers[0].g;
-    p.n_img = g0.n; p.h = g0.h_out; p.w = g0.w_out; p.rows0 = (p.h + 1) / 2; p.n_layers = n_layers;
+    p.n_img = g0.n; p.h = g0.h_out; p.w = g0.w_out; p.n_layers = n_layers;
+    p.cl = (p.h + CH_TILE_ROWS - 1) / CH_TILE_ROWS;
     p.sleep_ns = opts.sleep_ns;
     const StageGeom& gl = layers[n_layers - 1].g;
-    p.out = layers[n_layers - 1].out;
-    p.out_pitch = gl.out_pitch > 0 ? gl.out_pitch : gl.c_out;
-    for (int r = 0; r < 2; ++r) {
-        const int rows_local = r == 0 ? p.rows0 : p.h - p.rows0;
+    void* y = layers[n_layers - 1].out;
+    const int out_pitch = gl.out_pitch > 0 ? gl.out_pitch : gl.c_out;
+    for (int r = 0; r < p.cl; ++r) {
+        const int rows_local = std::min(CH_TILE_ROWS, p.h - CH_TILE_ROWS * r);
         int nz = 0;
         auto add = [&](int slot) {
             for (int i = 0; i < nz; ++i) if (p.zero_slots[r][i] == slot) return;
             p.zero_slots[r][nz++] = (unsigned char)slot;
         };
         for (int rr = 0; rr <= rows_local + 1; ++rr) { add(rr * CH_PITCH + p.w); add(rr * CH_PITCH + CH_PITCH - 1); }
-        const int border = r == 0 ? 0 : rows_local + 1;
-        for (int c = 0; c < p.w; ++c) add(border * CH_PITCH + c);
+        if (r == 0) for (int c = 0; c < p.w; ++c) add(c);
+        if (r == p.cl - 1) for (int c = 0; c < p.w; ++c) add((rows_local + 1) * CH_PITCH + c);
         p.n_zero[r] = nz;
     }
     const size_t es = 2;
@@ -450,7 +526,7 @@
         L.c_in = g.c_in; L.c_out = g.c_out;
         L.kblocks = (g.c_in + 63) / 64;
         L.n_pad = (g.c_out + 63) / 64 * 64;
-        L.np = (L.n_pad + 127) / 128;
+        L.ncw = (L.n_pad + CH_B_ROWS - 1) / CH_B_ROWS;
         L.aff_bytes = L.n_pad * 8;
         void* dwp = nullptr; float2* aff = nullptr;
         if (cudaMalloc(&dwp, (size_t)L.kblocks * CH_DWP) != cudaSuccess || cudaMalloc(&aff, (size_t)L.n_pad * sizeof(float2)) != cudaSuccess) {
@@ -466,7 +542,7 @@
         L.dwp = dwp; L.affine = aff;
         cuuint64_t dims[2] = {(cuuint64_t)g.c_in, (cuuint64_t)g.c_out};
         cuuint64_t strides[1] = {(cuuint64_t)g.c_in * es};
-        cuuint32_t box[2] = {64, 128};
+        cuuint32_t box[2] = {64, (cuuint32_t)CH_B_ROWS};
         cuuint32_t estr[2] = {1, 1};
         CUresult r = encode(&cp->maps.w[l], dt, 2, const_cast<void*>(layers[l].pw_w), dims, strides, box, estr, CU_TENSOR_MAP_INTERLEAVE_NONE,
                             CU_TENSOR_MAP_SWIZZLE_128B, CU_TENSOR_MAP_L2_PROMOTION_L2_256B, CU_TENSOR_MAP_FLOAT_OOB_FILL_NONE);
@@ -483,23 +559,25 @@
                             CU_TENSOR_MAP_SWIZZLE_128B, CU_TENSOR_MAP_L2_PROMOTION_L2_128B, CU_TENSOR_MAP_FLOAT_OOB_FILL_NONE);
         if (r != CUDA_SUCCESS) rc = fail(FD_ERR_CUDA, "cuTensorMapEncodeTiled(chain input) failed: " + std::to_string((int)r));
     }
-    for (int r = 0; r < 2 && rc == FD_OK; ++r) {
-        const int rows_r = r == 0 ? p.rows0 : p.h - p.rows0;
-        const cuuint64_t P = (cuuint64_t)p.out_pitch;
+    for (int r = 0; r < p.cl && rc == FD_OK; ++r) {
+        const int rows_r = std::min(CH_TILE_ROWS, p.h - CH_TILE_ROWS * r);
+        const cuuint64_t P = (cuuint64_t)out_pitch;
         cuuint64_t dims[4] = {(cuuint64_t)gl.c_out, (cuuint64_t)gl.w_out, (cuuint64_t)gl.h_out, (cuuint64_t)gl.n};
         cuuint64_t strides[3] = {P * es, (cuuint64_t)gl.w_out * P * es, (cuuint64_t)gl.h_out * gl.w_out * P * es};
         cuuint32_t box[4] = {64, (cuuint32_t)CH_PITCH, (cuuint32_t)rows_r, 1};
         cuuint32_t estr[4] = {1, 1, 1, 1};
-        CUresult cr = encode(&cp->maps.out[r], dt, 4, p.out, dims, strides, box, estr, CU_TENSOR_MAP_INTERLEAVE_NONE,
+        CUresult cr = encode(&cp->maps.out[r], dt, 4, y, dims, strides, box, estr, CU_TENSOR_MAP_INTERLEAVE_NONE,
                              CU_TENSOR_MAP_SWIZZLE_128B, CU_TENSOR_MAP_L2_PROMOTION_L2_128B, CU_TENSOR_MAP_FLOAT_OOB_FILL_NONE);
         if (cr != CUDA_SUCCESS) rc = fail(FD_ERR_CUDA, "cuTensorMapEncodeTiled(chain output) failed: " + std::to_string((int)cr));
     }
+    if (rc == FD_OK) {
+        if (dtype == FD_F16) rc = cp->relu6 ? chain_size_grid<__half, true>(cp) : chain_size_grid<__half, false>(cp);
+        else rc = cp->relu6 ? chain_size_grid<__nv_bfloat16, true>(cp) : chain_size_grid<__nv_bfloat16, false>(cp);
+    }
     if (rc != FD_OK) { chain_tc_destroy(cp); return rc; }
-    const int clusters = std::min(p.n_img, std::max(1, opts.n_sms / 2));
-    cp->grid = dim3((unsigned)(2 * clusters), 1, 1);
     char buf[160];
-    snprintf(buf, sizeof(buf), "chain_tc<k3,s1,2cta>[%d layers,%dx%d,c%d..%d,kb%d,smem%dK]", n_layers, p.h, p.w, p.L[0].c_in, p.L[n_layers - 1].c_out,
-             p.L[0].kblocks, CH_SMEM_BYTES / 1024);
+    snprintf(buf, sizeof(buf), "chain_tc<k3,s1,2cta>[%d layers,%dx%d,c%d..%d,kb%d,%dcta,smem%dK]", n_layers, p.h, p.w, p.L[0].c_in,
+             p.L[n_layers - 1].c_out, p.L[0].kblocks, p.cl, CH_SMEM_BYTES / 1024);
     cp->name = buf;
     *out = cp;
     return FD_OK;
@@ -507,21 +585,12 @@
 
 template <typename T, bool RELU6>
 static int chain_launch_inst(ChainTcPlan* cp, cudaStream_t st) {
-    auto kern = chain_tc_kernel<T, RELU6>;
-    static PerDeviceOnce attr_set;
-    int dev = -1;
-    FD_CUDA_OK(cudaGetDevice(&dev));
-    if (attr_set.need(dev)) {
-        FD_CUDA_OK(cudaFuncSetAttribute(kern, cudaFuncAttributeMaxDynamicSharedMemorySize, CH_SMEM_BYTES));
-        attr_set.done(dev);
-    }
-    cudaLaunchConfig_t cfg{};
-    cfg.gridDim = cp->grid; cfg.blockDim = dim3(CH_THREADS); cfg.dynamicSmemBytes = CH_SMEM_BYTES; cfg.stream = st;
-    cudaLaunchAttribute attr[1];
-    attr[0].id = cudaLaunchAttributeProgrammaticStreamSerialization;
-    attr[0].val.programmaticStreamSerializationAllowed = 1;
-    cfg.attrs = attr; cfg.numAttrs = cp->opts.pdl ? 1 : 0;
-    FD_CUDA_OK(cudaLaunchKernelEx(&cfg, kern, cp->maps, cp->p));
+    int rc = chain_kernel_ready<T, RELU6>();
+    if (rc != FD_OK) return rc;
+    cudaLaunchConfig_t cfg;
+    cudaLaunchAttribute attr[2];
+    chain_config(cp, st, cfg, attr);
+    FD_CUDA_OK(cudaLaunchKernelEx(&cfg, chain_tc_kernel<T, RELU6>, cp->maps, cp->p));
     FD_CUDA_OK(cudaGetLastError());
     return FD_OK;
 }
diff --git a/fastdepth_b200/plan.py b/fastdepth_b200/plan.py
--- a/fastdepth_b200/plan.py
+++ b/fastdepth_b200/plan.py
@@ -266,8 +266,8 @@
                 lo, hi = st['kernel'].split('{stages ')[1].rstrip('}').split('-')
                 in_chain = in_chain or int(lo) <= stage <= int(hi)
         if in_chain:
-            cnames = ('layer_start', 'dw_first_kb_computed', 'dw_done_grp0', 'pointwise_done', 'epilogue_done', 'local_barrier',
-                      'halo_received', 'mma_first_a_full', 'mma_last_pass_done', 'dw_done_grp1', 'tma_first_b_issue', 'unused11')
+            cnames = ('dw_layer_start', 'dw_input_ready', 'dw_first_kb_done', 'dw_done', 'mma_first_operands', 'mma_done',
+                      'consumers_met', 'epilogue_local_done', 'halo_sent', 'mma_done_wg1', 'tma_first_b_issue', 'layer_end')
             return {n: a[i][a[i] > 0] for i, n in enumerate(cnames)}
         names = ('tma_issue', 'dw_start', 'dw_math_done', 'a_published', 'mma_ready', 'mma_issued', 'unused6', 'epi_done',
                  'unused8', 'epi_staged', 'epi_barrier', 'epi_store_issued')
```

Result: slower. 57120, median of 6 (-2.0%).
